# emonosuke/emoASR

Measured on AMD Instinct MI355X. Metric: train frames/sec + decode RTF, Conformer-CTC 23M, 80-mel, 1/2/4/8 GPU, higher is better.
Workload: dtype bf16; 1 GPU; CTC(Conformer) 23M `L2`, bf16, SpecAugment on-GPU, synthetic LibriSpeech-shaped batches (2000 utts, lognormal lengths, ASRBatchSampler packing 30000 frames/50 utts per GPU), one step = accum_grad 5 micro-batches (the reference's accum_grad: 5, asr/train_asr.py:106-128, stacked through the engine in one pass) fwd+bwd, then all-reduce+clip+Adam; dropout 0.1; accum_grad=5, stacked_micro_batches=True, parallelism=dp1

## Files before the change

emoasr_amd/csrc/api.hip:

```cpp
#include <cstdarg>
#include <cstdio>
#include <cstring>
#include <map>
#include <mutex>
#include <tuple>
#include "common.h"
#include "../../include/emoasr_hip.h"

static thread_local char g_err[512] = "";

EmoScratch* emo_stream_scratch(int slot, void* stream, size_t bytes) {
  static std::mutex mu;
  static std::map<std::tuple<int, void*, int>, EmoScratch*> tab;
  int dev = 0;
  if (hipGetDevice(&dev) != hipSuccess) return nullptr;
  std::lock_guard<std::mutex> lock(mu);
  const auto key = std::make_tuple(dev, stream, slot);
  auto it = tab.find(key);
  if (it != tab.end() && it->second->bytes >= bytes) return it->second;
  hipStreamCaptureStatus cap = hipStreamCaptureStatusNone;
  if (hipStreamIsCapturing((hipStream_t)stream, &cap) != hipSuccess || cap != hipStreamCaptureStatusNone) {
    emo_set_error("stream scratch %d: first use on a stream that is being captured (run the call once eagerly on this stream)", slot);
    return nullptr;
  }
  void* d = nullptr;
  if (hipMalloc(&d, bytes) != hipSuccess || hipMemsetAsync(d, 0, bytes, (hipStream_t)stream) != hipSuccess) {
    emo_set_error("stream scratch %d: allocation of %zu bytes failed", slot, bytes);
    return nullptr;
  }
  EmoScratch* r = new EmoScratch{};
  r->dev = d; r->bytes = bytes;
  tab[key] = r;
  return r;
}

void emo_set_error(const char* fmt, ...) {
  va_list ap;
  va_start(ap, fmt);
  vsnprintf(g_err, sizeof(g_err), fmt, ap);
  va_end(ap);
}

void emo_gemm_set_tr_read(int v);
void emo_gemm_set_tile(int v);
void emo_gemm_set_tn_group_blocks(int v);
void emo_gemm_set_tn_group_kb(int v);
void emo_gemm_set_tn_place(int v);
void emo_gemm_set_tn_big(int v);
void emo_gemm_set_tn_big_blocks(int v);
void emo_gemm_set_wholek(int v);
void emo_gemm_set_kb(int v);
void emo_gemm_set_xcd(int v);
void emo_gemm_set_split_tile(int v);
void emo_gemm_set_split_kb(int v);
void emo_gemm_set_split_min128(int v);
void emo_gemm_set_conv_big(int v);
void emo_gemm_set_big_bm(int v);
void emo_gemm_set_big_korder(int v);
void emo_gemm_set_big_min_tiles(int v);
void emo_conv_set_dwconv_lds(int v);
void emo_layer_set_conv_fused(int v);
void emo_layer_set_wgrad_side(int v);
void emo_layer_set_stack_launch(int v);
void emo_layer_set_ffn_save_dact(int v);
void emo_layer_set_att_bits(int v);
void emo_ln_set_fwd8(int v);
void emo_gemm_set_wide128(int v);
void emo_gemm_set_big_n256(int v);
void emo_gemm_set_big_waves(int v);
void emo_conv1_set_pair(int v);
void emo_attn_set_prelaunch(int v);
void emo_ln_set_bwd_pf(int v);
void emo_ln_set_bwd_blocks(int v);
void emo_rnnt_set_greedy_coop(int v);
void emo_rnnt_set_beam_mfma(int v);
void emo_decode_set_coop(int v);
void emo_lstm_set_coop(int v);
void emo_decode_set_coop_merge(int v);
void emo_attn_set_tr_read(int v);
void emo_attn_set_fw(int v);
void emo_attn_set_fwd4(int v);
void emo_attn_set_q2(int v);
void emo_attn_set_bwd_split(int v);
void emo_attn_set_side(int v);
void emo_attn_set_side_prio(int v);
void emo_attn_set_lpt(int v);
void emo_attn_set_fwd_split(int v);
void emo_attn_set_xcd(int v);
void emo_attn_set_fwd_waves(int v);

#include <vector>
namespace {
const char* const kTimerNames[EMO_TIMER_COUNT] = {"attn_bwd_fused_kernel", "attn_bwd_dpos_kernel", "attn_fwd_kernel",
                                                  "gemm_tn_grouped_kernel", "gemm_nt_nn", "gemm_tn", "layernorm", "conv_module"};
struct TimerRec { hipEvent_t e0, e1; double flops, bytes; bool ended; };
std::vector<TimerRec> g_rec[EMO_TIMER_COUNT];
int g_timers_on = 0;
int g_timer_stride = 1;
long g_timer_seen[EMO_TIMER_COUNT];
bool g_timer_open[EMO_TIMER_COUNT];
bool timer_on(int id) { return g_timers_on == 1 || (g_timers_on > 1 && ((g_timers_on >> (id + 1)) & 1)); }
}
void emo_timer_begin(int id, hipStream_t s, double flops, double bytes) {
  if (!timer_on(id)) return;
  g_timer_open[id] = (g_timer_seen[id]++ % g_timer_stride) == 0;
  if (!g_timer_open[id]) return;
  TimerRec r{};
  hipEventCreate(&r.e0);
  hipEventCreate(&r.e1);
  hipEventRecord(r.e0, s);
  r.flops = flops; r.bytes = bytes; r.ended = false;
  g_rec[id].push_back(r);
}
void emo_timer_end(int id, hipStream_t s) {
  if (!timer_on(id) || !g_timer_open[id] || g_rec[id].empty() || g_rec[id].back().ended) return;
  hipEventRecord(g_rec[id].back().e1, s);
  g_rec[id].back().ended = true;
}
extern "C" int emoasr_timer_read_ex(const char* name, int* calls, double* ms, double* flops, double* bytes, int reset) {
  for (int id = 0; id < EMO_TIMER_COUNT; ++id) {
    if (strcmp(name, kTimerNames[id]) != 0) continue;
    double tot = 0.0, fl = 0.0, by = 0.0;
    int n = 0;
    for (const TimerRec& r : g_rec[id]) {
      if (!r.ended) continue;
      float t = 0.f;
      hipEventSynchronize(r.e1);
      if (hipEventElapsedTime(&t, r.e0, r.e1) == hipSuccess) { tot += t; fl += r.flops; by += r.bytes; ++n; }
    }
    if (calls) *calls = n;
    if (ms) *ms = tot;
    if (flops) *flops = fl;
    if (bytes) *bytes = by;
    if (reset) {
      for (const TimerRec& r : g_rec[id]) { hipEventDestroy(r.e0); hipEventDestroy(r.e1); }
      g_rec[id].clear();
    }
    return 0;
  }
  emo_set_error("unknown timer '%s'", name);
  return 1;
}
extern "C" int emoasr_timer_read(const char* name, int* calls, double* ms, int reset) {
  return emoasr_timer_read_ex(name, calls, ms, nullptr, nullptr, reset);
}

extern "C" const char* emoasr_last_error(void) { return g_err; }
extern "C" int emoasr_version(void) { return 1; }
extern "C" int emoasr_set_option(const char* name, int value) {
  if (strcmp(name, "tr_read") == 0) {
    emo_gemm_set_tr_read(value);
    emo_attn_set_tr_read(value);
    return 0;
  }
  if (strcmp(name, "gemm_tile") == 0) { emo_gemm_set_tile(value); return 0; }
  if (strcmp(name, "tn_group_blocks") == 0) { emo_gemm_set_tn_group_blocks(value); return 0; }
  if (strcmp(name, "tn_group_kb") == 0) { emo_gemm_set_tn_group_kb(value); return 0; }
  if (strcmp(name, "tn_place") == 0) { emo_gemm_set_tn_place(value); return 0; }
  if (strcmp(name, "tn_big") == 0) { emo_gemm_set_tn_big(value); return 0; }
  if (strcmp(name, "tn_big_blocks") == 0) { emo_gemm_set_tn_big_blocks(value); return 0; }
  if (strcmp(name, "gemm_wholek") == 0) { emo_gemm_set_wholek(value); return 0; }
  if (strcmp(name, "gemm_kb") == 0) { emo_gemm_set_kb(value); return 0; }
  if (strcmp(name, "gemm_xcd") == 0) { emo_gemm_set_xcd(value); return 0; }
  if (strcmp(name, "split_tile") == 0) { emo_gemm_set_split_tile(value); return 0; }
  if (strcmp(name, "split_kb") == 0) { emo_gemm_set_split_kb(value); return 0; }
  if (strcmp(name, "split_min128") == 0) { emo_gemm_set_split_min128(value); return 0; }
  if (strcmp(name, "conv_big") == 0) { emo_gemm_set_conv_big(value); return 0; }
  if (strcmp(name, "big_bm") == 0) { emo_gemm_set_big_bm(value); return 0; }
  if (strcmp(name, "big_korder") == 0) { emo_gemm_set_big_korder(value); return 0; }
  if (strcmp(name, "big_min_tiles") == 0) { emo_gemm_set_big_min_tiles(value); return 0; }
  if (strcmp(name, "dwconv_lds") == 0) { emo_conv_set_dwconv_lds(value); return 0; }
  if (strcmp(name, "conv_fused") == 0) { emo_layer_set_conv_fused(value); return 0; }
  if (strcmp(name, "wgrad_side") == 0) { emo_layer_set_wgrad_side(value); return 0; }
  if (strcmp(name, "stack_launch") == 0) { emo_layer_set_stack_launch(value); return 0; }
  if (strcmp(name, "ffn_save_dact") == 0) { emo_layer_set_ffn_save_dact(value); return 0; }
  if (strcmp(name, "attn_mask_bits") == 0) { emo_layer_set_att_bits(value); return 0; }
  if (strcmp(name, "attn_prelaunch") == 0) { emo_attn_set_prelaunch(value); return 0; }
  if (strcmp(name, "conv1_pair") == 0) { emo_conv1_set_pair(value); return 0; }
  if (strcmp(name, "big_waves") == 0) { emo_gemm_set_big_waves(value); return 0; }
  if (strcmp(name, "big_n256") == 0) { emo_gemm_set_big_n256(value); return 0; }
  if (strcmp(name, "gemm_wide128") == 0) { emo_gemm_set_wide128(value); return 0; }
  if (strcmp(name, "ln_fwd8") == 0) { emo_ln_set_fwd8(value); return 0; }
  if (strcmp(name, "ln_bwd_pf") == 0) { emo_ln_set_bwd_pf(value); return 0; }
  if (strcmp(name, "ln_bwd_blocks") == 0) { emo_ln_set_bwd_blocks(value); return 0; }
  if (strcmp(name, "rnnt_greedy_coop") == 0) { emo_rnnt_set_greedy_coop(value); return 0; }
  if (strcmp(name, "rnnt_beam_mfma") == 0) { emo_rnnt_set_beam_mfma(value); return 0; }
  if (strcmp(name, "decode_coop") == 0) { emo_decode_set_coop(value); return 0; }
  if (strcmp(name, "lstm_coop") == 0) { emo_lstm_set_coop(value); return 0; }
  if (strcmp(name, "decode_coop_merge") == 0) { emo_decode_set_coop_merge(value); return 0; }
  if (strcmp(name, "attn_fw") == 0) { emo_attn_set_fw(value); return 0; }
  if (strcmp(name, "attn_fwd4") == 0) { emo_attn_set_fwd4(value); return 0; }
  if (strcmp(name, "attn_q2") == 0) { emo_attn_set_q2(value); return 0; }
  if (strcmp(name, "attn_bwd_split") == 0) { emo_attn_set_bwd_split(value); return 0; }
  if (strcmp(name, "attn_side") == 0) { emo_attn_set_side(value); return 0; }
  if (strcmp(name, "attn_side_prio") == 0) { emo_attn_set_side_prio(value); return 0; }
  if (strcmp(name, "attn_lpt") == 0) { emo_attn_set_lpt(value); return 0; }
  if (strcmp(name, "attn_fwd_split") == 0) { emo_attn_set_fwd_split(value); return 0; }
  if (strcmp(name, "attn_xcd") == 0) { emo_attn_set_xcd(value); return 0; }
  if (strcmp(name, "attn_fwd_waves") == 0) { emo_attn_set_fwd_waves(value); return 0; }
  if (strcmp(name, "timers") == 0) { g_timers_on = value; return 0; }
  if (strcmp(name, "timer_stride") == 0) { g_timer_stride = value > 0 ? value : 1; return 0; }
  emo_set_error("unknown option '%s'", name);
  return 1;
}
```

emoasr_amd/csrc/convfused.hip:

```cpp
#include <algorithm>
#include "common.h"
#include "../../include/emoasr_hip.h"

namespace {

constexpr int CF_TT = 32;
constexpr int CF_MAXK = 31;
constexpr int CF_ROWS = CF_TT + CF_MAXK - 1;
constexpr int CF_CB = 256;
constexpr int CF_ROWS_P = 64;

typedef __attribute__((ext_vector_type(2))) float f2;
__device__ __forceinline__ f2 unpack2(unsigned u) { return f2{__uint_as_float(u << 16), __uint_as_float(u & 0xffff0000u)}; }
__device__ __forceinline__ unsigned pack2(f2 v) {
  const bf16 lo = (bf16)v[0], hi = (bf16)v[1];
  return (unsigned)__builtin_bit_cast(unsigned short, lo) | ((unsigned)__builtin_bit_cast(unsigned short, hi) << 16);
}
__device__ __forceinline__ unsigned lds_pair(const bf16* base, int row, int pair) {
  return *reinterpret_cast<const unsigned*>(base + row * CF_CB + 2 * pair);
}

template <bool GLU>
__global__ __launch_bounds__(CF_CB) void cf_dwconv_kernel(int Tn, int C, int K, const bf16* __restrict__ x,
                                                        const float* __restrict__ w, const float* __restrict__ bias,
                                                        bf16* __restrict__ y, int flip, float* __restrict__ part,
                                                        const RowSegs sg) {
  __shared__ __attribute__((aligned(16))) bf16 zs[CF_ROWS_P * CF_CB];
  __shared__ __attribute__((aligned(16))) bf16 os[CF_TT * CF_CB];
  const int tid = threadIdx.x;
  const int cb = blockIdx.y * CF_CB;
  const int ldx = GLU ? 2 * C : C;
  int b = blockIdx.z, nx = gridDim.x;
  if (sg.n > 1) {
    const int si = rowsegs_of_utt(sg, b);
    Tn = sg.T[si];
    x += sg.row[si] * ldx;
    y += sg.row[si] * C;
    if (part) part += sg.part[si];
    b -= sg.b0[si];
    nx = (Tn + CF_TT - 1) / CF_TT;
    if ((int)blockIdx.x >= nx) return;
  }
  const int t0 = blockIdx.x * CF_TT, pad = (K - 1) / 2;
  const int nch = min(CF_CB, C - cb);
  const int pr = tid & (CF_CB / 2 - 1), half = tid / (CF_CB / 2);
  f2 wr[CF_MAXK];
  {
    float* wsm = reinterpret_cast<float*>(zs);
    for (int idx = tid; idx < nch * K; idx += CF_CB) wsm[idx] = w[(long)cb * K + idx];
    __syncthreads();
#pragma unroll
    for (int j = 0; j < CF_MAXK; ++j) {
      const int jj = flip ? K - 1 - j : j;
      wr[j] = (j < K && 2 * pr < nch) ? f2{wsm[(2 * pr) * K + jj], wsm[(2 * pr + 1) * K + jj]} : f2{0.f, 0.f};
    }
    __syncthreads();
  }
  const __amdgpu_buffer_rsrc_t rs = make_rsrc(x + (long)b * Tn * ldx);
  const int ch8 = (tid & (CF_CB / 8 - 1)) * 8;
  {
    Vec16<bf16> sa[CF_ROWS_P / 8], sg[GLU ? CF_ROWS_P / 8 : 1];
#pragma unroll
    for (int it = 0; it < CF_ROWS_P / 8; ++it) {
      const int row = tid / (CF_CB / 8) + it * 8;
      const int t = t0 + row - pad;
      const bool ok = row < CF_TT + K - 1 && t >= 0 && t < Tn && ch8 < nch;
      const unsigned off = ok ? (unsigned)(((long)t * ldx + cb + ch8) * 2) : EMO_OOB;
      sa[it] = buf_load16<bf16>(rs, off);
      if constexpr (GLU) sg[it] = buf_load16<bf16>(rs, ok ? off + (unsigned)(C * 2) : EMO_OOB);
    }
#pragma unroll
    for (int it = 0; it < CF_ROWS_P / 8; ++it) {
      const int row = tid / (CF_CB / 8) + it * 8;
      Vec16<bf16> a = sa[it];
      if constexpr (GLU) {
#pragma unroll
        for (int e = 0; e < 8; ++e) a.v[e] = (bf16)((float)a.v[e] * sigmoidf_((float)sg[it].v[e]));
      }
      store16(&zs[row * CF_CB + ch8], a);
    }
  }
  __syncthreads();
  {
    const int c0 = cb + 2 * pr;
    if (2 * pr < nch) {
      const f2 bv = bias ? f2{bias[c0], bias[c0 + 1]} : f2{0.f, 0.f};
      f2 win[CF_TT / 2 + CF_MAXK - 1];
#pragma unroll
      for (int i = 0; i < CF_TT / 2 + CF_MAXK - 1; ++i) win[i] = unpack2(lds_pair(zs, half * (CF_TT / 2) + i, pr));
#pragma unroll
      for (int i = 0; i < CF_TT / 2; ++i) {
        f2 acc = bv;
#pragma unroll
        for (int j = 0; j < CF_MAXK; ++j) acc = emo_mac2(wr[j], win[i + j], acc);
        *reinterpret_cast<unsigned*>(os + (half * (CF_TT / 2) + i) * CF_CB + 2 * pr) = pack2(acc);
      }
    }
  }
  __syncthreads();
#pragma unroll
  for (int it = 0; it < CF_TT / 8; ++it) {
    const int row = tid / (CF_CB / 8) + it * 8;
    if (t0 + row < Tn && ch8 < nch)
      *reinterpret_cast<bf16x8*>(y + ((long)b * Tn + t0 + row) * C + cb + ch8) = *reinterpret_cast<const bf16x8*>(os + row * CF_CB + ch8);
  }
  if (part && tid < nch) {
    float out[CF_TT];
    float s = 0.f;
#pragma unroll
    for (int i = 0; i < CF_TT; ++i) {
      out[i] = t0 + i < Tn ? (float)os[i * CF_CB + tid] : 0.f;
      s += out[i];
    }
    const int n = min(CF_TT, Tn - t0);
    const float mb = s / n;
    float m2 = 0.f;
#pragma unroll
    for (int i = 0; i < CF_TT; ++i) {
      const float d = out[i] - mb;
      m2 += i < n ? d * d : 0.f;
    }
    float* p = part + ((long)b * nx + blockIdx.x) * 2 * C + cb + tid;
    p[0] = s;
    p[C] = m2;
  }
}

__global__ __launch_bounds__(CF_CB) void cf_conv_bwd_kernel(int Tn, int C, int K, const bf16* __restrict__ ds,
                                                          const bf16* __restrict__ cv, const float* __restrict__ mean,
                                                          const float* __restrict__ var, const float* __restrict__ gamma,
                                                          const float* __restrict__ beta, float eps,
                                                          const float* __restrict__ tot, const bf16* __restrict__ g,
                                                          const float* __restrict__ w, bf16* __restrict__ dg,
                                                          float* __restrict__ wpart, const RowSegs sg) {
  extern __shared__ __attribute__((aligned(16))) char smem[];
  bf16* dcs = reinterpret_cast<bf16*>(smem);
  bf16* zs = dcs + CF_ROWS_P * CF_CB;
  const int tid = threadIdx.x;
  const int cb = blockIdx.y * CF_CB;
  const int nch = min(CF_CB, C - cb);
  int b = blockIdx.z;
  if (sg.n > 1) {
    const int si = rowsegs_of_utt(sg, b);
    Tn = sg.T[si];
    ds += sg.row[si] * C; cv += sg.row[si] * C; g += sg.row[si] * 2 * C; dg += sg.row[si] * 2 * C;
    mean += (long)si * C; var += (long)si * C; tot += (long)si * 2 * C;
    b -= sg.b0[si];
    if ((int)blockIdx.x * CF_TT >= Tn) {
      float* p = wpart + ((long)blockIdx.z * gridDim.x + blockIdx.x) * (K + 1) * C + cb + tid;
      if (tid < nch)
        for (int j = 0; j <= K; ++j) p[(long)j * C] = 0.f;
      return;
    }
  }
  const int t0 = blockIdx.x * CF_TT, pad = (K - 1) / 2;
  const int ch8 = (tid & (CF_CB / 8 - 1)) * 8;
  const bool chok = ch8 < nch;
  const int pr = tid & (CF_CB / 2 - 1), half = tid / (CF_CB / 2);
  f2 wr[CF_MAXK];
  {
    float* wsm = reinterpret_cast<float*>(smem);
    for (int idx = tid; idx < nch * K; idx += CF_CB) wsm[idx] = w[(long)cb * K + idx];
    __syncthreads();
#pragma unroll
    for (int j = 0; j < CF_MAXK; ++j)
      wr[j] = (j < K && 2 * pr < nch) ? f2{wsm[(2 * pr) * K + (K - 1 - j)], wsm[(2 * pr + 1) * K + (K - 1 - j)]} : f2{0.f, 0.f};
    __syncthreads();
  }
  {
    const __amdgpu_buffer_rsrc_t rsd = make_rsrc(ds + (long)b * Tn * C), rsc = make_rsrc(cv + (long)b * Tn * C);
    const __amdgpu_buffer_rsrc_t rsg = make_rsrc(g + (long)b * Tn * 2 * C);
    {
      Vec16<bf16> ga[CF_ROWS_P / 8], gb[CF_ROWS_P / 8];
#pragma unroll
      for (int it = 0; it < CF_ROWS_P / 8; ++it) {
        const int row = tid / (CF_CB / 8) + it * 8;
        const int t = t0 + row - pad;
        const bool ok = row < CF_TT + K - 1 && t >= 0 && t < Tn && chok;
        const unsigned goff = ok ? (unsigned)(((long)t * 2 * C + cb + ch8) * 2) : EMO_OOB;
        ga[it] = buf_load16<bf16>(rsg, goff);
        gb[it] = buf_load16<bf16>(rsg, ok ? goff + (unsigned)(C * 2) : EMO_OOB);
      }
#pragma unroll
      for (int it = 0; it < CF_ROWS_P / 8; ++it) {
        const int row = tid / (CF_CB / 8) + it * 8;
        const int core = row - pad;
        (void)core;
        Vec16<bf16> z;
#pragma unroll
        for (int e = 0; e < 8; ++e) z.v[e] = (bf16)((float)ga[it].v[e] * sigmoidf_((float)gb[it].v[e]));
        store16(&zs[row * CF_CB + ch8], z);
      }
    }
    float mu[8], is[8], gm[8], bt[8], m1[8], m2[8];
#pragma unroll
    for (int j = 0; j < 8; ++j) {
      const int cc = cb + ch8 + j;
      mu[j] = chok ? mean[cc] : 0.f; is[j] = chok ? rsqrtf(var[cc] + eps) : 0.f;
      gm[j] = chok ? gamma[cc] : 0.f; bt[j] = chok ? beta[cc] : 0.f;
      m1[j] = chok ? tot[cc] : 0.f; m2[j] = chok ? tot[C + cc] : 0.f;
    }
    Vec16<bf16> dvs[CF_ROWS_P / 8], yvs[CF_ROWS_P / 8];
#pragma unroll
    for (int it = 0; it < CF_ROWS_P / 8; ++it) {
      const int row = tid / (CF_CB / 8) + it * 8;
      const int t = t0 + row - pad;
      const bool ok = row < CF_TT + K - 1 && t >= 0 && t < Tn && chok;
      const unsigned off = ok ? (unsigned)(((long)t * C + cb + ch8) * 2) : EMO_OOB;
      dvs[it] = buf_load16<bf16>(rsd, off);
      yvs[it] = buf_load16<bf16>(rsc, off);
    }
#pragma unroll
    for (int it = 0; it < CF_ROWS_P / 8; ++it) {
      const int row = tid / (CF_CB / 8) + it * 8;
      const int t = t0 + row - pad;
      const bool ok = row < CF_TT + K - 1 && t >= 0 && t < Tn && chok;
      const Vec16<bf16> dv = dvs[it], yv = yvs[it];
      Vec16<bf16> o;
#pragma unroll
      for (int e = 0; e < 8; ++e) {
        const float xh = ((float)yv.v[e] - mu[e]) * is[e];
        const float dbn = (float)dv.v[e] * dswishf_(gm[e] * xh + bt[e]);
        o.v[e] = ok ? (bf16)(gm[e] * is[e] * (dbn - m1[e] - xh * m2[e])) : (bf16)0.f;
      }
      store16(&dcs[row * CF_CB + ch8], o);
    }
  }
  __syncthreads();
  if (2 * pr >= nch) return;
  const int c0 = cb + 2 * pr;
  {
    f2 dcw[CF_TT / 2 + CF_MAXK - 1];
#pragma unroll
    for (int i = 0; i < CF_TT / 2 + CF_MAXK - 1; ++i) dcw[i] = unpack2(lds_pair(dcs, half * (CF_TT / 2) + i, pr));
    bf16* dgb = dg + (long)b * Tn * 2 * C + c0;
#pragma unroll
    for (int i = 0; i < CF_TT / 2; ++i) {
      f2 acc = f2{0.f, 0.f};
#pragma unroll
      for (int j = 0; j < CF_MAXK; ++j) acc = emo_mac2(wr[j], dcw[i + j], acc);
      const f2 d = unpack2(pack2(acc));
      const int fr = half * (CF_TT / 2) + i;
      const bool fok = t0 + fr < Tn;
      const bf16* gp = g + ((long)b * Tn + (fok ? t0 + fr : 0)) * 2 * C + c0;
      const f2 a = fok ? unpack2(*reinterpret_cast<const unsigned*>(gp)) : f2{0.f, 0.f};
      const f2 gt = fok ? unpack2(*reinterpret_cast<const unsigned*>(gp + C)) : f2{0.f, 0.f};
      const f2 sg = f2{sigmoidf_(gt[0]), sigmoidf_(gt[1])};
      if (t0 + fr < Tn) {
        *reinterpret_cast<unsigned*>(dgb + (long)(t0 + fr) * 2 * C) = pack2(d * sg);
        *reinterpret_cast<unsigned*>(dgb + (long)(t0 + fr) * 2 * C + C) = pack2(d * a * sg * (f2{1.f, 1.f} - sg));
      }
    }
  }
  {
    constexpr int TAPS = (CF_MAXK + 1) / 2;
    const int j0 = half * TAPS;
    f2 dcc[CF_TT];
#pragma unroll
    for (int i = 0; i < CF_TT; ++i) dcc[i] = unpack2(lds_pair(dcs, i + pad, pr));
    f2 zw[CF_TT + TAPS - 1];
#pragma unroll
    for (int i = 0; i < CF_TT + TAPS - 1; ++i) zw[i] = j0 + i < CF_ROWS_P ? unpack2(lds_pair(zs, j0 + i, pr)) : f2{0.f, 0.f};
    f2 acc[TAPS];
#pragma unroll
    for (int j = 0; j < TAPS; ++j) acc[j] = f2{0.f, 0.f};
    f2 sb = f2{0.f, 0.f};
#pragma unroll
    for (int i = 0; i < CF_TT; ++i) {
      const f2 d = dcc[i];
      sb += d;
#pragma unroll
      for (int j = 0; j < TAPS; ++j) acc[j] = emo_mac2(d, zw[i + j], acc[j]);
    }
    const long blk = ((long)blockIdx.z * gridDim.x + blockIdx.x);
    float* p = wpart + blk * (K + 1) * C + c0;
#pragma unroll
    for (int j = 0; j < TAPS; ++j)
      if (j0 + j < K) *reinterpret_cast<f2*>(p + (long)(j0 + j) * C) = acc[j];
    if (half == 0) *reinterpret_cast<f2*>(p + (long)K * C) = sb;
  }
}

}

int emo_dwconv_bwd_w_reduce(int nblk, int C, int K, const float* part, float* dw, float* dbias, hipStream_t s);

extern "C" int emoasr_glu_dwconv_fwd(int dtype, int B, int Tn, int C, int K, const void* g, const float* w,
                                     const float* bias, void* c, float* part, void* stream) {
  EMO_CHECK(dtype == EMO_BF16, "glu_dwconv_fwd: bf16 only");
  EMO_CHECK(K <= CF_MAXK && (K & 1) && C % 8 == 0, "glu_dwconv_fwd: K=%d (odd, <= %d), C=%d (multiple of 8)", K, CF_MAXK, C);
  EMO_CHECK((long)Tn * 2 * C * 2 < (1L << 32), "glu_dwconv_fwd: utterance larger than 4 GiB");
  if (B * Tn == 0) return 0;
  dim3 grid(cdiv(Tn, CF_TT), cdiv(C, CF_CB), B);
  cf_dwconv_kernel<true><<<grid, CF_CB, 0, (hipStream_t)stream>>>(Tn, C, K, (const bf16*)g, w, bias, (bf16*)c, 0, part, RowSegs{});
  EMO_LAUNCH_CHECK();
  return 0;
}

int emo_dwconv_lds(int B, int Tn, int C, int K, const void* x, const float* w, const float* bias, void* y, int flip,
                   float* part, hipStream_t s) {
  dim3 grid(cdiv(Tn, CF_TT), cdiv(C, CF_CB), B);
  cf_dwconv_kernel<false><<<grid, CF_CB, 0, s>>>(Tn, C, K, (const bf16*)x, w, bias, (bf16*)y, flip, part, RowSegs{});
  EMO_LAUNCH_CHECK();
  return 0;
}

extern "C" int emoasr_conv_bwd_fused(int dtype, int B, int Tn, int C, int K, const void* ds, const void* cv,
                                     const float* mean, const float* var, const float* gamma, const float* beta, float eps,
                                     const float* tot, const void* g, const float* w, void* dg, float* dw, float* dbias,
                                     float* scratch, void* stream) {
  EMO_CHECK(dtype == EMO_BF16, "conv_bwd_fused: bf16 only");
  EMO_CHECK(K <= CF_MAXK && (K & 1) && C % 8 == 0, "conv_bwd_fused: K=%d (odd, <= %d), C=%d (multiple of 8)", K, CF_MAXK, C);
  EMO_CHECK((long)Tn * 2 * C * 2 < (1L << 32), "conv_bwd_fused: utterance larger than 4 GiB");
  EMO_CHECK(scratch != nullptr && tot != nullptr, "conv_bwd_fused: scratch and tot are required");
  if (B * Tn == 0) return 0;
  hipStream_t s = (hipStream_t)stream;
  constexpr int bytes = 2 * CF_ROWS_P * CF_CB * 2;
  static bool attr_done = false;
  if (!attr_done) {
    hipError_t e = hipFuncSetAttribute((const void*)cf_conv_bwd_kernel, hipFuncAttributeMaxDynamicSharedMemorySize, bytes);
    if (e != hipSuccess) { emo_set_error("hipFuncSetAttribute(%d): %s", bytes, hipGetErrorString(e)); return 1; }
    attr_done = true;
  }
  dim3 grid(cdiv(Tn, CF_TT), cdiv(C, CF_CB), B);
  cf_conv_bwd_kernel<<<grid, CF_CB, bytes, s>>>(Tn, C, K, (const bf16*)ds, (const bf16*)cv, mean, var, gamma, beta, eps, tot,
                                              (const bf16*)g, w, (bf16*)dg, scratch, RowSegs{});
  EMO_LAUNCH_CHECK();
  return emo_dwconv_bwd_w_reduce(grid.x * B, C, K, scratch, dw, dbias, s);
}

int emo_bn_stats_finalize_seg(const RowSegs& sg, int C, const float* part, float* mean, float* var, float* running_mean,
                              float* running_var, float momentum, long long* nbt, hipStream_t s);
int emo_bn_swish_fwd_seg(const RowSegs& sg, int C, const void* y, const float* mean, const float* var, const float* gamma,
                         const float* beta, float eps, void* z, hipStream_t s);
int emo_bn_swish_bwd_sums_seg(const RowSegs& sg, int C, const void* dz, const void* y, const float* mean, const float* var,
                              const float* gamma, const float* beta, float eps, float* dgamma, float* dbeta, float* scratch,
                              float** tot_out, hipStream_t s);

namespace {
bool row_segs(const emoasr_segments_t* seg, int C, RowSegs* out, int* tmax) {
  if (!seg || seg->n < 1 || seg->n > EMOASR_MAX_SEGMENTS) return false;
  RowSegs sg{};
  sg.n = seg->n;
  *tmax = 0;
  for (int i = 0; i < seg->n; ++i) {
    if (seg->B[i] <= 0 || seg->T[i] <= 0) return false;
    sg.b0[i + 1] = sg.b0[i] + seg->B[i];
    sg.T[i] = seg->T[i];
    sg.row[i + 1] = sg.row[i] + (long)seg->B[i] * seg->T[i];
    sg.part[i + 1] = sg.part[i] + emoasr_dwconv_stats_floats(seg->B[i], seg->T[i], C);
    sg.sums[i + 1] = sg.sums[i] + (emoasr_bn_swish_bwd_scratch_floats(seg->B[i] * seg->T[i], C) / (2 * C) - 1);
    *tmax = std::max(*tmax, seg->T[i]);
  }
  *out = sg;
  return true;
}
}

extern "C" int emoasr_conv_module_fwd_seg(int dtype, const emoasr_segments_t* seg, int C, int K, const void* g, const float* w,
                                          const float* bias, void* c, float* part, float* bmean, float* bvar, float* running_mean,
                                          float* running_var, float momentum, long long* num_batches_tracked, const float* gamma,
                                          const float* beta, float eps, void* z, int training, void* stream) {
  EMO_CHECK(dtype == EMO_BF16, "conv_module_fwd_seg: bf16 only");
  EMO_CHECK(K <= CF_MAXK && (K & 1) && C % 8 == 0, "conv_module_fwd_seg: K=%d (odd, <= %d), C=%d (multiple of 8)", K, CF_MAXK, C);
  RowSegs sg;
  int tmax = 0;
  EMO_CHECK(row_segs(seg, C, &sg, &tmax), "conv_module_fwd_seg: bad segment description");
  EMO_CHECK((long)tmax * 2 * C * 2 < (1L << 32) && sg.row[sg.n] * 2 * C * 2 < (1L << 46), "conv_module_fwd_seg: batch too large");
  EMO_CHECK(!training || (part && bmean && bvar), "conv_module_fwd_seg: training needs the BatchNorm buffers");
  hipStream_t s = (hipStream_t)stream;
  EmoTimerScope timer_(EMO_TIMER_CONV_MODULE, s, 0.0, 5.0 * (double)sg.row[sg.n] * C * 2.0);
  dim3 grid(cdiv(tmax, CF_TT), cdiv(C, CF_CB), sg.b0[sg.n]);
  cf_dwconv_kernel<true><<<grid, CF_CB, 0, s>>>(tmax, C, K, (const bf16*)g, w, bias, (bf16*)c, 0, training ? part : nullptr, sg);
  EMO_LAUNCH_CHECK();
  if (training) {
    if (emo_bn_stats_finalize_seg(sg, C, part, bmean, bvar, running_mean, running_var, momentum, num_batches_tracked, s)) return 1;
    return emo_bn_swish_fwd_seg(sg, C, c, bmean, bvar, gamma, beta, eps, z, s);
  }
  RowSegs one{};
  one.n = 1; one.b0[1] = sg.b0[sg.n]; one.row[1] = sg.row[sg.n];
  return emo_bn_swish_fwd_seg(one, C, c, running_mean, running_var, gamma, beta, eps, z, s);
}

extern "C" long emoasr_conv_module_bwd_seg_scratch_floats(const emoasr_segments_t* seg, int C, int K, int which) {
  RowSegs sg;
  int tmax = 0;
  if (!row_segs(seg, C, &sg, &tmax)) return 0;
  if (which == 0) return (sg.sums[sg.n] + 2 * sg.n) * 2 * C;
  return emoasr_dwconv_bwd_w_scratch_floats(sg.b0[sg.n], tmax, C, K);
}

extern "C" int emoasr_conv_module_bwd_seg(int dtype, const emoasr_segments_t* seg, int C, int K, const void* dz, const void* c,
                                          const float* bmean, const float* bvar, const float* gamma, const float* beta, float eps,
                                          float* dgamma, float* dbeta, const void* g, const float* w, void* dg, float* dw,
                                          float* dbias, float* bn_scratch, float* dw_scratch, void* stream) {
  EMO_CHECK(dtype == EMO_BF16, "conv_module_bwd_seg: bf16 only");
  EMO_CHECK(K <= CF_MAXK && (K & 1) && C % 8 == 0, "conv_module_bwd_seg: K=%d (odd, <= %d), C=%d (multiple of 8)", K, CF_MAXK, C);
  EMO_CHECK(bn_scratch && dw_scratch, "conv_module_bwd_seg: scratch required");
  RowSegs sg;
  int tmax = 0;
  EMO_CHECK(row_segs(seg, C, &sg, &tmax), "conv_module_bwd_seg: bad segment description");
  hipStream_t s = (hipStream_t)stream;
  EmoTimerScope timer_(EMO_TIMER_CONV_MODULE, s, 0.0, 8.0 * (double)sg.row[sg.n] * C * 2.0);
  float* tot = nullptr;
  if (emo_bn_swish_bwd_sums_seg(sg, C, dz, c, bmean, bvar, gamma, beta, eps, dgamma, dbeta, bn_scratch, &tot, s)) return 1;
  constexpr int bytes = 2 * CF_ROWS_P * CF_CB * 2;
  static bool attr_done = false;
  if (!attr_done) {
    hipError_t e = hipFuncSetAttribute((const void*)cf_conv_bwd_kernel, hipFuncAttributeMaxDynamicSharedMemorySize, bytes);
    if (e != hipSuccess) { emo_set_error("hipFuncSetAttribute(%d): %s", bytes, hipGetErrorString(e)); return 1; }
    attr_done = true;
  }
  dim3 grid(cdiv(tmax, CF_TT), cdiv(C, CF_CB), sg.b0[sg.n]);
  cf_conv_bwd_kernel<<<grid, CF_CB, bytes, s>>>(tmax, C, K, (const bf16*)dz, (const bf16*)c, bmean, bvar, gamma, beta, eps, tot,
                                              (const bf16*)g, w, (bf16*)dg, dw_scratch, sg);
  EMO_LAUNCH_CHECK();
  return emo_dwconv_bwd_w_reduce(grid.x * sg.b0[sg.n], C, K, dw_scratch, dw, dbias, s);
}
```

emoasr_amd/csrc/convmodule.hip:

```cpp
#include <algorithm>
#include "common.h"
#include "../../include/emoasr_hip.h"

namespace {

constexpr int DW_TT = 32;
constexpr int DW_MAXK = 31;
constexpr int DW_WCHUNKS = 1;

template <typename T>
__global__ __launch_bounds__(256) void dwconv_kernel(int Tn, int C, int K, const T* __restrict__ x,
                                                     const float* __restrict__ w,
                                                     const float* __restrict__ bias, T* __restrict__ y,
                                                     int flip, float* __restrict__ part, const RowSegs sg) {
  const int c = blockIdx.y * 256 + threadIdx.x;
  if (c >= C) return;
  int b = blockIdx.z;
  if (sg.n > 1) {
    const int si = rowsegs_of_utt(sg, b);
    Tn = sg.T[si];
    x += sg.row[si] * C; y += sg.row[si] * C;
    if (part) part += sg.part[si];
    b -= sg.b0[si];
    if ((int)blockIdx.x * DW_TT >= Tn) return;
  }
  const int nx = (Tn + DW_TT - 1) / DW_TT;
  const int t0 = blockIdx.x * DW_TT, pad = (K - 1) / 2;
  float wr[DW_MAXK];
#pragma unroll
  for (int j = 0; j < DW_MAXK; ++j) wr[j] = j < K ? w[c * K + (flip ? K - 1 - j : j)] : 0.f;
  const float bv = bias ? bias[c] : 0.f;
  float win[DW_TT + DW_MAXK - 1];
  const __amdgpu_buffer_rsrc_t rs = make_rsrc(x + (long)b * Tn * C);
#pragma unroll
  for (int i = 0; i < DW_TT + DW_MAXK - 1; ++i) {
    const int t = t0 + i - pad;
    const bool ok = i < DW_TT + K - 1 && t >= 0 && t < Tn;
    win[i] = buf_load_f32<T>(rs, ok ? (unsigned)(((long)t * C + c) * sizeof(T)) : EMO_OOB);
  }
  T* yb = y + (long)b * Tn * C + c;
  float out[DW_TT];
  float s = 0.f;
#pragma unroll
  for (int i = 0; i < DW_TT; ++i) {
    float acc = bv;
#pragma unroll
    for (int j = 0; j < DW_MAXK; ++j) acc = emo_mac(wr[j], win[i + j], acc);
    const T r = from_f32<T>(acc);
    out[i] = t0 + i < Tn ? to_f32(r) : 0.f;
    s += out[i];
    if (t0 + i < Tn) yb[(long)(t0 + i) * C] = r;
  }
  if (part) {
    const int n = min(DW_TT, Tn - t0);
    const float mb = s / n;
    float m2 = 0.f;
#pragma unroll
    for (int i = 0; i < DW_TT; ++i) {
      const float d = out[i] - mb;
      m2 += i < n ? d * d : 0.f;
    }
    float* p = part + ((long)b * nx + blockIdx.x) * 2 * C + c;
    p[0] = s;
    p[C] = m2;
  }
}

constexpr int BNF_CH = 16, BNF_G = 64;
#define EMO_BN_TICKETS(stream_)                                                                   \
  EmoScratch* tsc_ = emo_stream_scratch(EMO_SCRATCH_BN_TICKETS, (void*)(stream_), 2 * 64 * sizeof(unsigned)); \
  if (!tsc_) return 1;                                                                            \
  unsigned* tickets_ = static_cast<unsigned*>(tsc_->dev)
__global__ __launch_bounds__(1024) void bn_stats_finalize_kernel(int B_, int Tn_, int C, const float* __restrict__ part_,
                                                                 float* __restrict__ mean_, float* __restrict__ var_,
                                                                 float* __restrict__ running_mean,
                                                                 float* __restrict__ running_var, float momentum,
                                                                 long long* __restrict__ num_batches_tracked, const RowSegs sg,
                                                                 unsigned* __restrict__ tickets) {
  __shared__ float red[BNF_G][BNF_CH];
  __shared__ float mean_s[BNF_CH];
  __shared__ int s_last;
  const int lane = threadIdx.x % BNF_CH, grp = threadIdx.x / BNF_CH;
  const int c = blockIdx.x * BNF_CH + lane;
  const int ns = sg.n > 1 ? sg.n : 1, si = blockIdx.y;
  const int B = sg.n > 1 ? sg.b0[si + 1] - sg.b0[si] : B_, Tn = sg.n > 1 ? sg.T[si] : Tn_;
  const float* part = sg.n > 1 ? part_ + sg.part[si] : part_;
  float* mean = mean_ + (long)si * C;
  float* var = var_ + (long)si * C;
  const int nx = (Tn + DW_TT - 1) / DW_TT, nblk = B * nx;
  const float M = (float)B * Tn;
  float s = 0.f;
  if (c < C) {
#pragma unroll 8
    for (int k = grp; k < nblk; k += BNF_G) s += part[(long)k * 2 * C + c];
  }
  red[grp][lane] = s;
  __syncthreads();
  if (grp == 0) {
    float t = 0.f;
#pragma unroll
    for (int g = 0; g < BNF_G; ++g) t += red[g][lane];
    mean_s[lane] = t / M;
  }
  __syncthreads();
  const float mu = mean_s[lane];
  float m2 = 0.f;
  if (c < C)
#pragma unroll 8
    for (int k = grp; k < nblk; k += BNF_G) {
      const int n = min(DW_TT, Tn - (k % nx) * DW_TT);
      const float d = part[(long)k * 2 * C + c] / n - mu;
      m2 += part[(long)k * 2 * C + C + c] + n * d * d;
    }
  __syncthreads();
  red[grp][lane] = m2;
  __syncthreads();
  float m2sum = 0.f;
  if (grp == 0 && c < C) {
#pragma unroll
    for (int g = 0; g < BNF_G; ++g) m2sum += red[g][lane];
    mean[c] = mu;
    var[c] = m2sum / M;
  }
  if (!running_mean && !running_var && !num_batches_tracked) return;
  __syncthreads();
  if (threadIdx.x == 0) {
    __threadfence();
    s_last = atomicAdd(&tickets[blockIdx.x], 1u) == (unsigned)ns - 1;
  }
  __syncthreads();
  if (!s_last) return;
  __threadfence();
  if (grp == 0 && c < C) {
    float rm = running_mean ? running_mean[c] : 0.f, rv = running_var ? running_var[c] : 0.f;
    for (int k = 0; k < ns; ++k) {
      const float Mk = sg.n > 1 ? (float)(sg.row[k + 1] - sg.row[k]) : M;
      const float mk = __hip_atomic_load(mean_ + (long)k * C + c, __ATOMIC_RELAXED, __HIP_MEMORY_SCOPE_AGENT);
      const float vk = __hip_atomic_load(var_ + (long)k * C + c, __ATOMIC_RELAXED, __HIP_MEMORY_SCOPE_AGENT);
      const float m2k = k == si ? m2sum : vk * Mk;
      rm = (1.f - momentum) * rm + momentum * (k == si ? mu : mk);
      rv = (1.f - momentum) * rv + momentum * (Mk > 1.f ? m2k / (Mk - 1.f) : m2k / Mk);
    }
    if (running_mean) running_mean[c] = rm;
    if (running_var) running_var[c] = rv;
  }
  if (threadIdx.x == 0) {
    tickets[blockIdx.x] = 0u;
    if (num_batches_tracked && blockIdx.x == 0) *num_batches_tracked += ns;
  }
}

template <typename T>
__global__ __launch_bounds__(256) void dwconv_bwd_w_kernel(int Tn, int C, int K, const T* __restrict__ dy,
                                                           const T* __restrict__ x, float* __restrict__ part, const RowSegs sg) {
  const int c = blockIdx.y * 256 + threadIdx.x;
  if (c >= C) return;
  int b = blockIdx.z;
  const int pad = (K - 1) / 2;
  if (sg.n > 1) {
    const int si = rowsegs_of_utt(sg, b);
    Tn = sg.T[si];
    x += sg.row[si] * C; dy += sg.row[si] * C;
    b -= sg.b0[si];
  }
  float acc[DW_MAXK];
#pragma unroll
  for (int j = 0; j < DW_MAXK; ++j) acc[j] = 0.f;
  float sb = 0.f;
  const __amdgpu_buffer_rsrc_t rsx = make_rsrc(x + (long)b * Tn * C), rsd = make_rsrc(dy + (long)b * Tn * C);
  for (int cc = 0; cc < DW_WCHUNKS; ++cc) {
    const int t0 = (blockIdx.x * DW_WCHUNKS + cc) * DW_TT;
    if (t0 >= Tn) break;
    float win[DW_TT + DW_MAXK - 1];
#pragma unroll
    for (int i = 0; i < DW_TT + DW_MAXK - 1; ++i) {
      const int t = t0 + i - pad;
      const bool ok = i < DW_TT + K - 1 && t >= 0 && t < Tn;
      win[i] = buf_load_f32<T>(rsx, ok ? (unsigned)(((long)t * C + c) * sizeof(T)) : EMO_OOB);
    }
    float dv[DW_TT];
#pragma unroll
    for (int i = 0; i < DW_TT; ++i)
      dv[i] = buf_load_f32<T>(rsd, t0 + i < Tn ? (unsigned)(((long)(t0 + i) * C + c) * sizeof(T)) : EMO_OOB);
#pragma unroll
    for (int i = 0; i < DW_TT; ++i) {
      const float d = dv[i];
      sb += d;
#pragma unroll
      for (int j = 0; j < DW_MAXK; ++j) acc[j] = emo_mac(d, win[i + j], acc[j]);
    }
  }
  const long blk = ((long)blockIdx.z * gridDim.x + blockIdx.x);
  float* p = part + blk * (K + 1) * C + c;
#pragma unroll
  for (int j = 0; j < DW_MAXK; ++j)
    if (j < K) p[(long)j * C] = acc[j];
  p[(long)K * C] = sb;
}

__global__ __launch_bounds__(256) void dwconv_bwd_w_reduce_kernel(int nblk, int C, int K,
                                                                  const float* __restrict__ part,
                                                                  float* __restrict__ dw,
                                                                  float* __restrict__ dbias) {
  __shared__ float red[4][64];
  const int lane = threadIdx.x & 63, wave = threadIdx.x >> 6;
  const int i = blockIdx.x * 64 + lane;
  const int n = (K + 1) * C;
  const int per = (nblk + gridDim.y - 1) / gridDim.y;
  const int b0 = blockIdx.y * per, b1 = min(nblk, b0 + per);
  float s = 0.f;
  if (i < n) {
#pragma unroll 8
    for (int b = b0 + wave; b < b1; b += 4) s += part[(long)b * n + i];
  }
  red[wave][lane] = s;
  __syncthreads();
  if (wave == 0 && i < n) {
    s = red[0][lane] + red[1][lane] + red[2][lane] + red[3][lane];
    const int j = i / C, c = i % C;
    if (gridDim.y == 1) {
      if (j < K) dw[c * K + j] += s;
      else if (dbias) dbias[c] += s;
    } else {
      if (j < K) atomicAdd(&dw[c * K + j], s);
      else if (dbias) atomicAdd(&dbias[c], s);
    }
  }
}

constexpr int BN_ROWS = 16;
constexpr int BN_STAT_ROWS = 64;
template <typename T>
__global__ __launch_bounds__(256) void bn_sum_kernel(int M, int C, const T* __restrict__ y,
                                                     float* __restrict__ sum) {
  const int c = blockIdx.x * 256 + threadIdx.x;
  if (c >= C) return;
  const int r0 = blockIdx.y * BN_STAT_ROWS, r1 = min(M, r0 + BN_STAT_ROWS);
  float s = 0.f;
  for (int r = r0; r < r1; ++r) s += to_f32(y[(long)r * C + c]);
  atomicAdd(&sum[c], s);
}
template <typename T>
__global__ __launch_bounds__(256) void bn_var_kernel(int M, int C, const T* __restrict__ y,
                                                     const float* __restrict__ sum,
                                                     float* __restrict__ sq) {
  const int c = blockIdx.x * 256 + threadIdx.x;
  if (c >= C) return;
  const float mu = sum[c] / M;
  const int r0 = blockIdx.y * BN_STAT_ROWS, r1 = min(M, r0 + BN_STAT_ROWS);
  float s = 0.f;
  for (int r = r0; r < r1; ++r) { const float d = to_f32(y[(long)r * C + c]) - mu; s += d * d; }
  atomicAdd(&sq[c], s);
}
__global__ void bn_finalize_kernel(int M, int C, float* mean, float* var, float* running_mean,
                                   float* running_var, float momentum) {
  const int c = blockIdx.x * 256 + threadIdx.x;
  if (c >= C) return;
  const float mu = mean[c] / M, vb = var[c] / M;
  mean[c] = mu; var[c] = vb;
  if (running_mean) running_mean[c] = (1.f - momentum) * running_mean[c] + momentum * mu;
  if (running_var) {
    const float vu = M > 1 ? var[c] * M / (M - 1) : vb;
    running_var[c] = (1.f - momentum) * running_var[c] + momentum * vu;
  }
}

template <typename T>
__global__ __launch_bounds__(256) void bn_swish_fwd_kernel(long n, int C, const T* __restrict__ y,
                                                           const float* __restrict__ mean,
                                                           const float* __restrict__ var,
                                                           const float* __restrict__ gamma,
                                                           const float* __restrict__ beta, float eps,
                                                           T* __restrict__ z, const RowSegs sg) {
  for (long i = (long)blockIdx.x * 256 + threadIdx.x; i < n; i += (long)gridDim.x * 256) {
    const int c = i % C;
    const long so = sg.n > 1 ? (long)rowsegs_of_row(sg, i / C) * C : 0;
    const float xh = (to_f32(y[i]) - mean[so + c]) * rsqrtf(var[so + c] + eps);
    z[i] = from_f32<T>(swish_t<T>(gamma[c] * xh + beta[c]));
  }
}
template <typename T>
__global__ __launch_bounds__(256) void bn_swish_fwd8_kernel(long n8, int C, const T* __restrict__ y,
                                                            const float* __restrict__ mean,
                                                            const float* __restrict__ var,
                                                            const float* __restrict__ gamma,
                                                            const float* __restrict__ beta, float eps,
                                                            T* __restrict__ z, const RowSegs sg) {
  const int cg = C / 8;
  for (long i = (long)blockIdx.x * 256 + threadIdx.x; i < n8; i += (long)gridDim.x * 256) {
    const long row = i / cg;
    const int c = (int)(i - row * cg) * 8;
    const long so = sg.n > 1 ? (long)rowsegs_of_row(sg, row) * C : 0;
    float v[8];
    load8<T>(y + i * 8, v);
#pragma unroll
    for (int j = 0; j < 8; ++j) {
      const float xh = (v[j] - mean[so + c + j]) * rsqrtf(var[so + c + j] + eps);
      v[j] = swish_t<T>(gamma[c + j] * xh + beta[c + j]);
    }
    store8<T>(z + i * 8, v);
  }
}

constexpr int BN_SUM_ROWS = 64;
constexpr int BN_APPLY_ROWS = 16;

template <typename T>
__global__ __launch_bounds__(256) void bn_bwd_sums_kernel(int M, int C, const T* __restrict__ dz,
                                                          const T* __restrict__ y,
                                                          const float* __restrict__ mean,
                                                          const float* __restrict__ var,
                                                          const float* __restrict__ gamma,
                                                          const float* __restrict__ beta, float eps,
                                                          float* __restrict__ part, const RowSegs sg) {
  __shared__ float red[8][2][256];
  const int hl = threadIdx.x & 31, rl = threadIdx.x >> 5;
  const int c = blockIdx.x * 256 + hl * 8;
  const bool cok = c < C;
  long rbase = 0;
  if (sg.n > 1) {
    const int si = blockIdx.z;
    rbase = sg.row[si];
    M = (int)(sg.row[si + 1] - rbase);
    if ((int)blockIdx.y * BN_SUM_ROWS >= M) return;
    mean += (long)si * C; var += (long)si * C;
    part += sg.sums[si] * 2 * C;
  }
  float mu[8], is[8], g[8], bt[8], s1[8], s2[8];
#pragma unroll
  for (int j = 0; j < 8; ++j) {
    mu[j] = cok ? mean[c + j] : 0.f; is[j] = cok ? rsqrtf(var[c + j] + eps) : 0.f;
    g[j] = cok ? gamma[c + j] : 0.f; bt[j] = cok ? beta[c + j] : 0.f;
    s1[j] = 0.f; s2[j] = 0.f;
  }
  const __amdgpu_buffer_rsrc_t rsy = make_rsrc(y), rsd = make_rsrc(dz);
  const int r0 = blockIdx.y * BN_SUM_ROWS;
#pragma unroll 4
  for (int it = 0; it < BN_SUM_ROWS / 8; ++it) {
    const int r = r0 + rl + 8 * it;
    const bool ok = cok && r < M;
    float yv[8], dv[8];
    buf_load8<T>(rsy, (rbase + r) * C + c, ok, yv);
    buf_load8<T>(rsd, (rbase + r) * C + c, ok, dv);
#pragma unroll
    for (int j = 0; j < 8; ++j) {
      const float xh = (yv[j] - mu[j]) * is[j];
      const float dbn = dv[j] * dswish_t<T>(g[j] * xh + bt[j]);
      s1[j] += dbn; s2[j] += dbn * xh;
    }
  }
#pragma unroll
  for (int j = 0; j < 8; ++j) { red[rl][0][hl * 8 + j] = s1[j]; red[rl][1][hl * 8 + j] = s2[j]; }
  __syncthreads();
  const int cc = blockIdx.x * 256 + threadIdx.x;
  if (cc < C) {
    float a = 0.f, b = 0.f;
#pragma unroll
    for (int k = 0; k < 8; ++k) { a += red[k][0][threadIdx.x]; b += red[k][1][threadIdx.x]; }
    part[(long)blockIdx.y * 2 * C + cc] = a;
    part[(long)blockIdx.y * 2 * C + C + cc] = b;
  }
}
__global__ __launch_bounds__(1024) void bn_bwd_fold_kernel(int npart_, int C, float inv_m_, const float* __restrict__ part_,
                                                           float* __restrict__ tot_, float* __restrict__ dgamma,
                                                           float* __restrict__ dbeta, const RowSegs sg,
                                                           unsigned* __restrict__ tickets) {
  __shared__ float red[2][64][16];
  __shared__ int s_last;
  const int lane = threadIdx.x % 16, grp = threadIdx.x / 16;
  const int c = blockIdx.x * 16 + lane;
  const int ns = sg.n > 1 ? sg.n : 1, si = blockIdx.y;
  const int npart = sg.n > 1 ? (int)(sg.sums[si + 1] - sg.sums[si]) : npart_;
  const float inv_m = sg.n > 1 ? 1.f / (float)(sg.row[si + 1] - sg.row[si]) : inv_m_;
  const float* part = sg.n > 1 ? part_ + sg.sums[si] * 2 * C : part_;
  float* tot = tot_ + (long)si * 2 * C;
  float* raw = tot_ + (long)ns * 2 * C + (long)si * 2 * C;
  float a = 0.f, b = 0.f;
  if (c < C) {
#pragma unroll 8
    for (int k = grp; k < npart; k += 64) { a += part[(long)k * 2 * C + c]; b += part[(long)k * 2 * C + C + c]; }
  }
  red[0][grp][lane] = a;
  red[1][grp][lane] = b;
  __syncthreads();
  if (grp == 0 && c < C) {
    a = 0.f; b = 0.f;
#pragma unroll
    for (int g = 0; g < 64; ++g) { a += red[0][g][lane]; b += red[1][g][lane]; }
    tot[c] = a * inv_m;
    tot[C + c] = b * inv_m;
    if (ns == 1) {
      if (dbeta) dbeta[c] += a;
      if (dgamma) dgamma[c] += b;
    } else {
      raw[c] = a;
      raw[C + c] = b;
    }
  }
  if (ns == 1 || (!dbeta && !dgamma)) return;
  __syncthreads();
  if (threadIdx.x == 0) {
    __threadfence();
    s_last = atomicAdd(&tickets[64 + blockIdx.x], 1u) == (unsigned)ns - 1;
  }
  __syncthreads();
  if (!s_last) return;
  __threadfence();
  if (grp == 0 && c < C) {
    float da = 0.f, db = 0.f;
    const float* r0 = tot_ + (long)ns * 2 * C;
    for (int k = 0; k < ns; ++k) {
      da += __hip_atomic_load(r0 + (long)k * 2 * C + c, __ATOMIC_RELAXED, __HIP_MEMORY_SCOPE_AGENT);
      db += __hip_atomic_load(r0 + (long)k * 2 * C + C + c, __ATOMIC_RELAXED, __HIP_MEMORY_SCOPE_AGENT);
    }
    if (dbeta) dbeta[c] += da;
    if (dgamma) dgamma[c] += db;
  }
  if (threadIdx.x == 0) tickets[64 + blockIdx.x] = 0u;
}
template <typename T>
__global__ __launch_bounds__(256) void bn_bwd_apply_kernel(int M, int C, const T* __restrict__ dz,
                                                           const T* __restrict__ y,
                                                           const float* __restrict__ mean,
                                                           const float* __restrict__ var,
                                                           const float* __restrict__ gamma,
                                                           const float* __restrict__ beta, float eps,
                                                           const float* __restrict__ tot,
                                                           T* __restrict__ dy, const RowSegs sg) {
  const int hl = threadIdx.x & 31, rl = threadIdx.x >> 5;
  const int c = blockIdx.x * 256 + hl * 8;
  if (c >= C) return;
  if (sg.n > 1) {
    const int si = blockIdx.z;
    M = (int)(sg.row[si + 1] - sg.row[si]);
    if ((int)blockIdx.y * BN_APPLY_ROWS >= M) return;
    dz += sg.row[si] * C; y += sg.row[si] * C; dy += sg.row[si] * C;
    mean += (long)si * C; var += (long)si * C; tot += (long)si * 2 * C;
  }
  float mu[8], is[8], g[8], bt[8], m1[8], m2[8];
#pragma unroll
  for (int j = 0; j < 8; ++j) {
    mu[j] = mean[c + j]; is[j] = rsqrtf(var[c + j] + eps); g[j] = gamma[c + j]; bt[j] = beta[c + j];
    m1[j] = tot[c + j]; m2[j] = tot[C + c + j];
  }
  const __amdgpu_buffer_rsrc_t rsy = make_rsrc(y), rsd = make_rsrc(dz);
  const int r0 = blockIdx.y * BN_APPLY_ROWS;
#pragma unroll
  for (int it = 0; it < BN_APPLY_ROWS / 8; ++it) {
    const int r = r0 + rl + 8 * it;
    const bool ok = r < M;
    float yv[8], dv[8], o[8];
    buf_load8<T>(rsy, (long)r * C + c, ok, yv);
    buf_load8<T>(rsd, (long)r * C + c, ok, dv);
#pragma unroll
    for (int j = 0; j < 8; ++j) {
      const float xh = (yv[j] - mu[j]) * is[j];
      const float dbn = dv[j] * dswish_t<T>(g[j] * xh + bt[j]);
      o[j] = g[j] * is[j] * (dbn - m1[j] - xh * m2[j]);
    }
    if (ok) store8<T>(dy + (long)r * C + c, o);
  }
}

inline int ew_grid(long n) { long b = (n + 255) / 256; return (int)(b > 8192 ? 8192 : (b < 1 ? 1 : b)); }

}

int emo_dwconv_lds(int B, int Tn, int C, int K, const void* x, const float* w, const float* bias, void* y, int flip,
                   float* part, hipStream_t s);
static int g_dwconv_lds = 1;
void emo_conv_set_dwconv_lds(int v) { g_dwconv_lds = v; }
static bool use_lds(int dtype, int Tn, int C) {
  return g_dwconv_lds && dtype == EMO_BF16 && C % 8 == 0 && (long)Tn * C * 2 < (1L << 32);
}
int emo_dwconv_bwd_w_reduce(int nblk, int C, int K, const float* part, float* dw, float* dbias, hipStream_t s) {
  dwconv_bwd_w_reduce_kernel<<<dim3(cdiv((K + 1) * C, 64), nblk >= 1024 ? 4 : 1), 256, 0, s>>>(nblk, C, K, part, dw, dbias);
  EMO_LAUNCH_CHECK();
  return 0;
}

extern "C" int emoasr_dwconv_fwd(int dtype, int B, int Tn, int C, int K, const void* x, const float* w,
                                 const float* bias, void* y, void* stream) {
  EMO_CHECK(K <= DW_MAXK && (K & 1), "dwconv: K=%d unsupported (odd, <= %d)", K, DW_MAXK);
  if (B * Tn == 0) return 0;
  if (use_lds(dtype, Tn, C)) return emo_dwconv_lds(B, Tn, C, K, x, w, bias, y, 0, nullptr, (hipStream_t)stream);
  dim3 grid(cdiv(Tn, DW_TT), cdiv(C, 256), B);
  EMO_DISPATCH(dtype, (dwconv_kernel<T><<<grid, 256, 0, (hipStream_t)stream>>>(Tn, C, K, (const T*)x, w,
                                                                              bias, (T*)y, 0, nullptr, RowSegs{})));
  EMO_LAUNCH_CHECK();
  return 0;
}

extern "C" long emoasr_dwconv_stats_floats(int B, int Tn, int C) { return (long)B * cdiv(Tn, DW_TT) * 2 * C; }

extern "C" int emoasr_dwconv_fwd_stats(int dtype, int B, int Tn, int C, int K, const void* x, const float* w,
                                       const float* bias, void* y, float* part, void* stream) {
  EMO_CHECK(K <= DW_MAXK && (K & 1), "dwconv: K=%d unsupported", K);
  EMO_CHECK(part != nullptr && B * Tn > 0, "dwconv_fwd_stats: needs a non-empty batch and the partials buffer");
  if (use_lds(dtype, Tn, C)) return emo_dwconv_lds(B, Tn, C, K, x, w, bias, y, 0, part, (hipStream_t)stream);
  dim3 grid(cdiv(Tn, DW_TT), cdiv(C, 256), B);
  EMO_DISPATCH(dtype, (dwconv_kernel<T><<<grid, 256, 0, (hipStream_t)stream>>>(Tn, C, K, (const T*)x, w,
                                                                              bias, (T*)y, 0, part, RowSegs{})));
  EMO_LAUNCH_CHECK();
  return 0;
}

extern "C" int emoasr_bn_stats_finalize(int B, int Tn, int C, const float* part, float* mean, float* var,
                                        float* running_mean, float* running_var, float momentum,
                                        long long* num_batches_tracked, void* stream) {
  EMO_CHECK(B * Tn > 0, "bn_stats_finalize: empty batch");
  EMO_CHECK(cdiv(C, BNF_CH) <= 64, "bn_stats_finalize: C=%d too wide for the ticket table", C);
  EMO_BN_TICKETS(stream);
  bn_stats_finalize_kernel<<<cdiv(C, BNF_CH), 1024, 0, (hipStream_t)stream>>>(B, Tn, C, part, mean, var, running_mean,
                                                                          running_var, momentum, num_batches_tracked, RowSegs{}, tickets_);
  EMO_LAUNCH_CHECK();
  return 0;
}
extern "C" int emoasr_dwconv_bwd_x(int dtype, int B, int Tn, int C, int K, const void* dy, const float* w,
                                   void* dx, void* stream) {
  EMO_CHECK(K <= DW_MAXK && (K & 1), "dwconv: K=%d unsupported", K);
  if (B * Tn == 0) return 0;
  if (use_lds(dtype, Tn, C)) return emo_dwconv_lds(B, Tn, C, K, dy, w, nullptr, dx, 1, nullptr, (hipStream_t)stream);
  dim3 grid(cdiv(Tn, DW_TT), cdiv(C, 256), B);
  EMO_DISPATCH(dtype, (dwconv_kernel<T><<<grid, 256, 0, (hipStream_t)stream>>>(Tn, C, K, (const T*)dy, w,
                                                                              nullptr, (T*)dx, 1, nullptr, RowSegs{})));
  EMO_LAUNCH_CHECK();
  return 0;
}
extern "C" long emoasr_dwconv_bwd_w_scratch_floats(int B, int Tn, int C, int K) {
  return (long)B * cdiv(Tn, DW_TT * DW_WCHUNKS) * (K + 1) * C;
}

extern "C" int emoasr_dwconv_bwd_w(int dtype, int B, int Tn, int C, int K, const void* dy, const void* x,
                                   float* dw, float* dbias, int accumulate, float* scratch, void* stream) {
  EMO_CHECK(K <= DW_MAXK && (K & 1), "dwconv: K=%d unsupported", K);
  hipStream_t s = (hipStream_t)stream;
  if (!accumulate) {
    hipMemsetAsync(dw, 0, sizeof(float) * C * K, s);
    if (dbias) hipMemsetAsync(dbias, 0, sizeof(float) * C, s);
  }
  if (B * Tn == 0) return 0;
  EMO_CHECK(scratch != nullptr, "dwconv_bwd_w: scratch of emoasr_dwconv_bwd_w_scratch_floats() floats required");
  dim3 grid(cdiv(Tn, DW_TT * DW_WCHUNKS), cdiv(C, 256), B);
  EMO_DISPATCH(dtype, (dwconv_bwd_w_kernel<T><<<grid, 256, 0, s>>>(Tn, C, K, (const T*)dy, (const T*)x, scratch, RowSegs{})));
  const int nblk = grid.x * B;
  dwconv_bwd_w_reduce_kernel<<<cdiv((K + 1) * C, 64), 256, 0, s>>>(nblk, C, K, scratch, dw, dbias);
  EMO_LAUNCH_CHECK();
  return 0;
}

extern "C" int emoasr_bn_stats(int dtype, int M, int C, const void* y, float* mean, float* var,
                               float* running_mean, float* running_var, float momentum, void* stream) {
  EMO_CHECK(M > 0, "bn_stats: empty batch");
  hipStream_t s = (hipStream_t)stream;
  hipMemsetAsync(mean, 0, sizeof(float) * C, s);
  hipMemsetAsync(var, 0, sizeof(float) * C, s);
  dim3 grid(cdiv(C, 256), cdiv(M, BN_STAT_ROWS));
  EMO_DISPATCH(dtype, (bn_sum_kernel<T><<<grid, 256, 0, s>>>(M, C, (const T*)y, mean)));
  EMO_DISPATCH(dtype, (bn_var_kernel<T><<<grid, 256, 0, s>>>(M, C, (const T*)y, mean, var)));
  bn_finalize_kernel<<<cdiv(C, 256), 256, 0, s>>>(M, C, mean, var, running_mean, running_var, momentum);
  EMO_LAUNCH_CHECK();
  return 0;
}

extern "C" int emoasr_bn_swish_fwd(int dtype, int M, int C, const void* y, const float* mean,
                                   const float* var, const float* gamma, const float* beta, float eps,
                                   void* z, void* stream) {
  const long n = (long)M * C;
  if (n == 0) return 0;
  if (C % 8 == 0 && (reinterpret_cast<uintptr_t>(y) | reinterpret_cast<uintptr_t>(z)) % 16 == 0) {
    EMO_DISPATCH(dtype, (bn_swish_fwd8_kernel<T><<<ew_grid(n / 8), 256, 0, (hipStream_t)stream>>>(
                            n / 8, C, (const T*)y, mean, var, gamma, beta, eps, (T*)z, RowSegs{})));
  } else {
    EMO_DISPATCH(dtype, (bn_swish_fwd_kernel<T><<<ew_grid(n), 256, 0, (hipStream_t)stream>>>(
                            n, C, (const T*)y, mean, var, gamma, beta, eps, (T*)z, RowSegs{})));
  }
  EMO_LAUNCH_CHECK();
  return 0;
}

extern "C" long emoasr_bn_swish_bwd_scratch_floats(int M, int C) { return ((long)cdiv(M, BN_SUM_ROWS) + 1) * 2 * C; }

extern "C" int emoasr_bn_swish_bwd_sums(int dtype, int M, int C, const void* dz, const void* y, const float* mean,
                                        const float* var, const float* gamma, const float* beta, float eps,
                                        float* dgamma, float* dbeta, float* scratch, float** tot_out, void* stream) {
  EMO_CHECK(M > 0, "bn_swish_bwd_sums: empty batch");
  hipStream_t s = (hipStream_t)stream;
  EMO_CHECK(C % 8 == 0, "bn_swish_bwd_sums: C=%d must be a multiple of 8", C);
  EMO_CHECK((long)M * C * (dtype == EMO_BF16 ? 2 : 4) < (1L << 32), "bn_swish_bwd_sums: activation larger than 4 GiB");
  const int npart = cdiv(M, BN_SUM_ROWS);
  dim3 sgrid(cdiv(C, 256), npart);
  EMO_DISPATCH(dtype, (bn_bwd_sums_kernel<T><<<sgrid, 256, 0, s>>>(M, C, (const T*)dz, (const T*)y, mean,
                                                                  var, gamma, beta, eps, scratch, RowSegs{})));
  float* tot = scratch + (long)npart * 2 * C;
  EMO_BN_TICKETS(s);
  bn_bwd_fold_kernel<<<cdiv(C, 16), 1024, 0, s>>>(npart, C, 1.f / M, scratch, tot, dgamma, dbeta, RowSegs{}, tickets_);
  if (tot_out) *tot_out = tot;
  EMO_LAUNCH_CHECK();
  return 0;
}

extern "C" int emoasr_bn_swish_bwd(int dtype, int M, int C, const void* dz, const void* y,
                                   const float* mean, const float* var, const float* gamma,
                                   const float* beta, float eps, void* dy, float* dgamma, float* dbeta,
                                   float* scratch, void* stream) {
  EMO_CHECK(M > 0, "bn_swish_bwd: empty batch");
  hipStream_t s = (hipStream_t)stream;
  EMO_CHECK(C % 8 == 0, "bn_swish_bwd: C=%d must be a multiple of 8", C);
  EMO_CHECK((long)M * C * (dtype == EMO_BF16 ? 2 : 4) < (1L << 32), "bn_swish_bwd: activation larger than 4 GiB");
  const int npart = cdiv(M, BN_SUM_ROWS);
  dim3 grid(cdiv(C, 256), cdiv(M, BN_APPLY_ROWS));
  dim3 sgrid(cdiv(C, 256), npart);
  EMO_DISPATCH(dtype, (bn_bwd_sums_kernel<T><<<sgrid, 256, 0, s>>>(M, C, (const T*)dz, (const T*)y, mean,
                                                                  var, gamma, beta, eps, scratch, RowSegs{})));
  float* tot = scratch + (long)npart * 2 * C;
  EMO_BN_TICKETS(s);
  bn_bwd_fold_kernel<<<cdiv(C, 16), 1024, 0, s>>>(npart, C, 1.f / M, scratch, tot, dgamma, dbeta, RowSegs{}, tickets_);
  EMO_DISPATCH(dtype, (bn_bwd_apply_kernel<T><<<grid, 256, 0, s>>>(M, C, (const T*)dz, (const T*)y, mean,
                                                                  var, gamma, beta, eps, tot, (T*)dy, RowSegs{})));
  EMO_LAUNCH_CHECK();
  return 0;
}

int emo_bn_stats_finalize_seg(const RowSegs& sg, int C, const float* part, float* mean, float* var, float* running_mean,
                              float* running_var, float momentum, long long* nbt, hipStream_t s) {
  EMO_CHECK(cdiv(C, BNF_CH) <= 64, "bn_stats_finalize: C=%d too wide for the ticket table", C);
  EMO_BN_TICKETS(s);
  bn_stats_finalize_kernel<<<dim3(cdiv(C, BNF_CH), sg.n > 1 ? sg.n : 1), 1024, 0, s>>>(sg.b0[1], sg.T[0], C, part, mean, var,
                                                                                     running_mean, running_var, momentum, nbt, sg, tickets_);
  EMO_LAUNCH_CHECK();
  return 0;
}

int emo_bn_swish_fwd_seg_dt(int dtype, const RowSegs& sg, int C, const void* y, const float* mean, const float* var,
                            const float* gamma, const float* beta, float eps, void* z, hipStream_t s) {
  const long n = sg.row[sg.n] * C;
  if (n == 0) return 0;
  if (C % 8 == 0) {
    EMO_DISPATCH(dtype, (bn_swish_fwd8_kernel<T><<<ew_grid(n / 8), 256, 0, s>>>(n / 8, C, (const T*)y, mean, var, gamma, beta, eps, (T*)z, sg)));
  } else {
    EMO_DISPATCH(dtype, (bn_swish_fwd_kernel<T><<<ew_grid(n), 256, 0, s>>>(n, C, (const T*)y, mean, var, gamma, beta, eps, (T*)z, sg)));
  }
  EMO_LAUNCH_CHECK();
  return 0;
}
int emo_bn_swish_fwd_seg(const RowSegs& sg, int C, const void* y, const float* mean, const float* var, const float* gamma,
                         const float* beta, float eps, void* z, hipStream_t s) {
  return emo_bn_swish_fwd_seg_dt(EMO_BF16, sg, C, y, mean, var, gamma, beta, eps, z, s);
}
int emo_bn_bwd_apply(int dtype, int M, int C, const void* dz, const void* y, const float* mean, const float* var, const float* gamma,
                     const float* beta, float eps, const float* tot, void* dy, hipStream_t s) {
  dim3 grid(cdiv(C, 256), cdiv(M, BN_APPLY_ROWS));
  EMO_DISPATCH(dtype, (bn_bwd_apply_kernel<T><<<grid, 256, 0, s>>>(M, C, (const T*)dz, (const T*)y, mean, var, gamma, beta, eps, tot, (T*)dy, RowSegs{})));
  EMO_LAUNCH_CHECK();
  return 0;
}
int emo_bn_bwd_apply_seg(int dtype, const RowSegs& sg, int C, const void* dz, const void* y, const float* mean, const float* var,
                         const float* gamma, const float* beta, float eps, const float* tot, void* dy, hipStream_t s) {
  long mmax = 0;
  for (int i = 0; i < sg.n; ++i) mmax = std::max(mmax, sg.row[i + 1] - sg.row[i]);
  dim3 grid(cdiv(C, 256), cdiv((int)mmax, BN_APPLY_ROWS), sg.n);
  EMO_DISPATCH(dtype, (bn_bwd_apply_kernel<T><<<grid, 256, 0, s>>>((int)mmax, C, (const T*)dz, (const T*)y, mean, var, gamma, beta, eps,
                                                                  tot, (T*)dy, sg)));
  EMO_LAUNCH_CHECK();
  return 0;
}
int emo_dwconv_seg(int dtype, const RowSegs& sg, int tmax, int C, int K, const void* x, const float* w, const float* bias, void* y,
                   int flip, float* part, hipStream_t s) {
  EMO_CHECK(K <= DW_MAXK && (K & 1), "dwconv: K=%d unsupported (odd, <= %d)", K, DW_MAXK);
  if (sg.b0[sg.n] == 0 || tmax == 0) return 0;
  dim3 grid(cdiv(tmax, DW_TT), cdiv(C, 256), sg.b0[sg.n]);
  EMO_DISPATCH(dtype, (dwconv_kernel<T><<<grid, 256, 0, s>>>(tmax, C, K, (const T*)x, w, bias, (T*)y, flip, part, sg)));
  EMO_LAUNCH_CHECK();
  return 0;
}
int emo_dwconv_bwd_w_seg(int dtype, const RowSegs& sg, int tmax, int C, int K, const void* dy, const void* x, float* dw, float* dbias,
                         float* scratch, hipStream_t s) {
  EMO_CHECK(K <= DW_MAXK && (K & 1), "dwconv: K=%d unsupported", K);
  if (sg.b0[sg.n] == 0 || tmax == 0) return 0;
  EMO_CHECK(scratch != nullptr, "dwconv_bwd_w_seg: scratch of emoasr_dwconv_bwd_w_scratch_floats(all utterances, longest) floats required");
  dim3 grid(cdiv(tmax, DW_TT * DW_WCHUNKS), cdiv(C, 256), sg.b0[sg.n]);
  EMO_DISPATCH(dtype, (dwconv_bwd_w_kernel<T><<<grid, 256, 0, s>>>(tmax, C, K, (const T*)dy, (const T*)x, scratch, sg)));
  const int nblk = grid.x * sg.b0[sg.n];
  dwconv_bwd_w_reduce_kernel<<<dim3(cdiv((K + 1) * C, 64), nblk >= 1024 ? 4 : 1), 256, 0, s>>>(nblk, C, K, scratch, dw, dbias);
  EMO_LAUNCH_CHECK();
  return 0;
}

int emo_bn_swish_bwd_sums_seg_dt(int dtype, const RowSegs& sg, int C, const void* dz, const void* y, const float* mean, const float* var,
                                 const float* gamma, const float* beta, float eps, float* dgamma, float* dbeta, float* scratch,
                                 float** tot_out, hipStream_t s);
int emo_bn_swish_bwd_sums_seg(const RowSegs& sg, int C, const void* dz, const void* y, const float* mean, const float* var,
                              const float* gamma, const float* beta, float eps, float* dgamma, float* dbeta, float* scratch,
                              float** tot_out, hipStream_t s) {
  return emo_bn_swish_bwd_sums_seg_dt(EMO_BF16, sg, C, dz, y, mean, var, gamma, beta, eps, dgamma, dbeta, scratch, tot_out, s);
}
int emo_bn_swish_bwd_sums_seg_dt(int dtype, const RowSegs& sg, int C, const void* dz, const void* y, const float* mean, const float* var,
                                 const float* gamma, const float* beta, float eps, float* dgamma, float* dbeta, float* scratch,
                                 float** tot_out, hipStream_t s) {
  long mmax = 0;
  for (int i = 0; i < sg.n; ++i) mmax = std::max(mmax, sg.row[i + 1] - sg.row[i]);
  EMO_CHECK(sg.row[sg.n] * C * (dtype == EMO_BF16 ? 2 : 4) < (1L << 32), "bn_swish_bwd_sums_seg: activation larger than 4 GiB");
  dim3 sgrid(cdiv(C, 256), cdiv((int)mmax, BN_SUM_ROWS), sg.n);
  EMO_DISPATCH(dtype, (bn_bwd_sums_kernel<T><<<sgrid, 256, 0, s>>>((int)mmax, C, (const T*)dz, (const T*)y, mean, var, gamma, beta, eps,
                                                                  scratch, sg)));
  float* tot = scratch + sg.sums[sg.n] * 2 * C;
  EMO_CHECK(cdiv(C, 16) <= 64, "bn_swish_bwd_sums_seg: C=%d too wide for the ticket table", C);
  EMO_BN_TICKETS(s);
  bn_bwd_fold_kernel<<<dim3(cdiv(C, 16), sg.n > 1 ? sg.n : 1), 1024, 0, s>>>((int)sg.sums[1], C, 1.f / (float)sg.row[1], scratch, tot,
                                                                         dgamma, dbeta, sg, tickets_);
  if (tot_out) *tot_out = tot;
  EMO_LAUNCH_CHECK();
  return 0;
}
```

emoasr_amd/csrc/layer.hip:

```cpp
#include <math.h>
#include <algorithm>
#include <map>
#include <mutex>
#include <utility>
#include "common.h"
#include "../../include/emoasr_hip.h"

void emo_attn_bwd_fused_extras(float* zero, long zn, const float* cast_src, void* cast_dst, long cn);
void emo_attn_bwd_defer_join(int v);
void emo_attn_bwd_join(void* stream);
int emo_attn_bwd_prelaunch(int dtype, const emoasr_attn_t* a, void* ws, size_t ws_bytes, float* zero, long zn, void* stream);

int emo_bn_stats_finalize_seg(const RowSegs& sg, int C, const float* part, float* mean, float* var, float* running_mean,
                              float* running_var, float momentum, long long* nbt, hipStream_t s);
int emo_bn_swish_fwd_seg_dt(int dtype, const RowSegs& sg, int C, const void* y, const float* mean, const float* var,
                            const float* gamma, const float* beta, float eps, void* z, hipStream_t s);
int emo_bn_swish_bwd_sums_seg_dt(int dtype, const RowSegs& sg, int C, const void* dz, const void* y, const float* mean, const float* var,
                                 const float* gamma, const float* beta, float eps, float* dgamma, float* dbeta, float* scratch,
                                 float** tot_out, hipStream_t s);
int emo_bn_bwd_apply_seg(int dtype, const RowSegs& sg, int C, const void* dz, const void* y, const float* mean, const float* var,
                         const float* gamma, const float* beta, float eps, const float* tot, void* dy, hipStream_t s);
int emo_dwconv_seg(int dtype, const RowSegs& sg, int tmax, int C, int K, const void* x, const float* w, const float* bias, void* y,
                   int flip, float* part, hipStream_t s);
int emo_dwconv_bwd_w_seg(int dtype, const RowSegs& sg, int tmax, int C, int K, const void* dy, const void* x, float* dw, float* dbias,
                         float* scratch, hipStream_t s);

namespace {

emoasr_epilogue_t plain_ep() {
  emoasr_epilogue_t e{};
  e.alpha = 1.f;
  e.res_scale = 1.f;
  return e;
}

int g_att_bits = 1;
int g_ffn_save_dact = 1;
int g_stack_launch = 1;
int g_conv_fused = 1;
bool conv_fused_ok(int dtype, int d) { return g_conv_fused && dtype == EMO_BF16 && d % 8 == 0; }

int g_wgrad_side = 0;
struct WgSide {
  hipStream_t side = nullptr;
  hipEvent_t fork = nullptr, done[2] = {nullptr, nullptr};
  bool pending[2] = {false, false};
  unsigned n = 0;
};
std::mutex g_wg_mu;
std::map<std::pair<int, hipStream_t>, WgSide> g_wg;

WgSide* wg_side_of(hipStream_t s, bool create) {
  hipStreamCaptureStatus cap = hipStreamCaptureStatusNone;
  if (hipStreamIsCapturing(s, &cap) != hipSuccess || cap != hipStreamCaptureStatusNone) return nullptr;
  int dev = 0;
  if (hipGetDevice(&dev) != hipSuccess) return nullptr;
  std::lock_guard<std::mutex> lk(g_wg_mu);
  auto it = g_wg.find({dev, s});
  if (it != g_wg.end()) return &it->second;
  if (!create) return nullptr;
  WgSide w;
  if (hipStreamCreateWithFlags(&w.side, hipStreamNonBlocking) != hipSuccess) return nullptr;
  if (hipEventCreateWithFlags(&w.fork, hipEventDisableTiming) != hipSuccess ||
      hipEventCreateWithFlags(&w.done[0], hipEventDisableTiming) != hipSuccess ||
      hipEventCreateWithFlags(&w.done[1], hipEventDisableTiming) != hipSuccess)
    return nullptr;
  return &(g_wg[{dev, s}] = w);
}

int ffn_fwd(int dtype, int M, int d, int F, const emoasr_ffn_params_t& p, const void* x, float res_scale,
            float p_enc, uint64_t s_in, uint64_t s_out, const emoasr_ffn_stash_t& st, void* stream) {
  if (emoasr_layernorm_fwd(dtype, M, d, x, p.ln_g, p.ln_b, 1e-5f, st.h, st.mean, st.rstd, stream)) return 1;
  emoasr_epilogue_t e1 = plain_ep();
  e1.bias = p.b1; e1.act = EMOASR_ACT_SWISH | (g_ffn_save_dact ? EMOASR_ACT_SAVE_DACT : 0); e1.pre_out = st.u; e1.drop_p = p_enc; e1.seed = s_in;
  if (emoasr_gemm_nt(dtype, M, F, d, st.h, d, p.w1, d, st.a, F, &e1, stream)) return 1;
  emoasr_epilogue_t e2 = plain_ep();
  e2.bias = p.b2; e2.residual = x; e2.ldr = d; e2.res_scale = res_scale; e2.drop_p = p_enc; e2.seed = s_out;
  return emoasr_gemm_nt(dtype, M, d, F, st.a, F, p.w2, F, st.y, d, &e2, stream);
}

struct SegView {
  int n = 0, Btot = 0;
  int B[EMOASR_MAX_SEGMENTS], T[EMOASR_MAX_SEGMENTS], b0[EMOASR_MAX_SEGMENTS];
  long row[EMOASR_MAX_SEGMENTS + 1], prow[EMOASR_MAX_SEGMENTS + 1], part[EMOASR_MAX_SEGMENTS + 1];
  long M() const { return row[n]; }
  long R() const { return prow[n]; }
};

bool seg_view(const emoasr_conformer_fwd_t* io, int d, SegView* v) {
  const emoasr_segments_t& s = io->seg;
  if (s.n < 0 || s.n > EMOASR_MAX_SEGMENTS) return false;
  v->n = s.n > 0 ? s.n : 1;
  v->row[0] = v->prow[0] = v->part[0] = 0;
  v->Btot = 0;
  for (int i = 0; i < v->n; ++i) {
    v->B[i] = s.n > 0 ? s.B[i] : io->B;
    v->T[i] = s.n > 0 ? s.T[i] : io->T;
    if (v->B[i] <= 0 || v->T[i] <= 0) return false;
    v->b0[i] = v->Btot;
    v->Btot += v->B[i];
    v->row[i + 1] = v->row[i] + (long)v->B[i] * v->T[i];
    v->prow[i + 1] = v->prow[i] + 2L * v->T[i] - 1;
    v->part[i + 1] = v->part[i] + emoasr_dwconv_stats_floats(v->B[i], v->T[i], d);
  }
  return true;
}

RowSegs row_segs_of(const SegView& sv, int C) {
  RowSegs sg{};
  sg.n = sv.n;
  for (int i = 0; i < sv.n; ++i) {
    sg.b0[i + 1] = sg.b0[i] + sv.B[i];
    sg.T[i] = sv.T[i];
    sg.row[i + 1] = sv.row[i + 1];
    sg.part[i + 1] = sv.part[i + 1];
    sg.sums[i + 1] = sg.sums[i] + (emoasr_bn_swish_bwd_scratch_floats(sv.B[i] * sv.T[i], C) / (2 * C) - 1);
  }
  return sg;
}

void attn_args_for(emoasr_attn_t& a, const SegView& sv, int s0, int s1, int H, int d, size_t esz, const void* qkv, const void* pp,
                   const int* klens, uint64_t seed) {
  const size_t ro = (size_t)sv.row[s0];
  const char* base = (const char*)qkv + ro * 3 * d * esz;
  int nb = 0, tmax = 0;
  for (int k = s0; k < s1; ++k) { nb += sv.B[k]; tmax = std::max(tmax, sv.T[k]); }
  a.B = nb; a.H = H; a.DK = d / H; a.Tq = tmax; a.Tk = tmax;
  a.ldq = a.ldk = a.ldv = 3 * d; a.ldo = d; a.ldp = d;
  a.q = base; a.k = base + (size_t)d * esz; a.v = base + (size_t)2 * d * esz;
  a.pos = (const char*)pp + (size_t)sv.prow[s0] * d * esz;
  a.klens = klens ? klens + sv.b0[s0] : nullptr;
  a.causal = 0; a.scale = 1.f / sqrtf((float)(d / H));
  a.seed = seed + 0x9E3779B97F4A7C15ull * (uint64_t)s0;
  a.nseg = 0;
  if (s1 - s0 > 1) {
    a.nseg = s1 - s0;
    for (int k = s0; k <= s1; ++k) {
      a.seg_b0[k - s0] = k < s1 ? sv.b0[k] - sv.b0[s0] : nb;
      a.seg_row[k - s0] = sv.row[k] - sv.row[s0];
      a.seg_prow[k - s0] = sv.prow[k] - sv.prow[s0];
      if (k < s1) a.seg_T[k - s0] = sv.T[k];
    }
  }
}

}

void emo_layer_set_wgrad_side(int v) { g_wgrad_side = v ? 1 : 0; }
extern "C" int emoasr_wgrad_side_join(int keep, void* stream) {
  hipStream_t s = (hipStream_t)stream;
  WgSide* w = wg_side_of(s, false);
  if (!w) return 0;
  for (int back = 2; back > (keep > 0 ? 1 : 0); --back) {
    if (w->n < (unsigned)back) continue;
    const int slot = (w->n - back) & 1;
    if (!w->pending[slot]) continue;
    if (hipStreamWaitEvent(s, w->done[slot], 0) != hipSuccess) { emo_set_error("wgrad_side_join: hipStreamWaitEvent failed"); return 1; }
    w->pending[slot] = false;
  }
  return 0;
}
void emo_layer_set_conv_fused(int v) { g_conv_fused = v; }
void emo_layer_set_stack_launch(int v) { g_stack_launch = v; }
void emo_layer_set_ffn_save_dact(int v) { g_ffn_save_dact = v ? 1 : 0; }
void emo_layer_set_att_bits(int v) { g_att_bits = v ? 1 : 0; }

extern "C" int emoasr_conformer_attn_masks(int dtype, int nl, const emoasr_segments_t* seg, int B, int T, int H, int d, const int* klens,
                                           float p_att, const uint64_t* seeds, unsigned* masks, long layer_stride_words, int nw,
                                           void* stream) {
  EMO_CHECK(seg && seeds && masks && nl >= 0 && H > 0 && d % H == 0, "conformer_attn_masks: bad arguments");
  if (p_att <= 0.f) return 0;
  emoasr_conformer_fwd_t io{};
  io.B = B; io.T = T; io.seg = *seg;
  SegView sv;
  EMO_CHECK(seg_view(&io, d, &sv), "conformer_attn_masks: bad batch / segment shapes");
  const size_t esz = dtype == EMO_BF16 ? 2 : 4;
  const int astep = g_stack_launch ? sv.n : 1;
  for (int l = 0; l < nl; ++l)
    for (int si = 0; si < sv.n; si += astep) {
      emoasr_attn_t am{};
      attn_args_for(am, sv, si, si + astep, H, d, esz, nullptr, nullptr, klens, seeds[l]);
      am.drop_p = p_att;
      if (emoasr_attn_dropmask(dtype, &am, masks + (size_t)l * layer_stride_words + (size_t)sv.row[si] * H * nw, nw, stream)) return 1;
    }
  return 0;
}

extern "C" int emoasr_conformer_layer_fwd(int dtype, const emoasr_conformer_layer_t* L,
                                          const emoasr_conformer_fwd_t* io, void* stream) {
  EMO_CHECK(L && io && io->x && io->pos_t, "conformer_layer_fwd: missing arguments");
  const int d = L->d, H = L->H, F = L->F;
  EMO_CHECK(d > 0 && H > 0 && d % H == 0, "conformer_layer_fwd: bad dims d=%d H=%d", d, H);
  SegView sv;
  EMO_CHECK(seg_view(io, d, &sv), "conformer_layer_fwd: bad batch / segment shapes (B=%d T=%d segments=%d)", io->B, io->T, io->seg.n);
  const int M = (int)sv.M(), R = (int)sv.R();
  const size_t esz = dtype == EMO_BF16 ? 2 : 4;
  const float p_enc = io->p_enc;
  const bool att_bits = g_att_bits && io->att_mask && io->training && io->p_att > 0.f && dtype == EMO_BF16;
  const int astep_m = g_stack_launch ? sv.n : 1;
  for (int si = 0; si < sv.n && att_bits && !io->att_mask_ready; si += astep_m) {
    emoasr_attn_t am{};
    attn_args_for(am, sv, si, si + astep_m, H, d, esz, io->qkv, io->pp, io->klens, io->seed[2]);
    am.drop_p = io->p_att;
    if (emoasr_attn_dropmask(dtype, &am, io->att_mask + (size_t)sv.row[si] * H * io->att_mask_nw, io->att_mask_nw, stream)) return 1;
  }
  if (ffn_fwd(dtype, M, d, F, L->ffm, io->x, 0.5f, p_enc, io->seed[0], io->seed[1], io->ffm, stream)) return 1;
  const void* x1 = io->ffm.y;
  if (emoasr_layernorm_fwd(dtype, M, d, x1, L->att_ln_g, L->att_ln_b, 1e-5f, io->at_h, io->at_mean, io->at_rstd, stream))
    return 1;
  {
    emoasr_epilogue_t e = plain_ep();
    e.bias = L->bqkv;
    if (emoasr_gemm_nt(dtype, M, 3 * d, d, io->at_h, d, L->wqkv, d, io->qkv, 3 * d, &e, stream)) return 1;
    emoasr_epilogue_t ep = plain_ep();
    if (emoasr_gemm_nt(dtype, R, d, d, io->pos_t, d, L->wpos, d, io->pp, d, &ep, stream)) return 1;
    const int astep = g_stack_launch ? sv.n : 1;
    for (int si = 0; si < sv.n; si += astep) {
      const size_t ro = (size_t)sv.row[si];
      emoasr_attn_t a{};
      attn_args_for(a, sv, si, si + astep, H, d, esz, io->qkv, io->pp, io->klens, io->seed[2]);
      a.bias_u = L->bias_u; a.bias_v = L->bias_v; a.drop_p = io->p_att;
      a.out = (char*)io->o + ro * d * esz; a.lse = io->lse + ro * H;
      if (att_bits) { a.keep_mask = io->att_mask + ro * H * io->att_mask_nw; a.keep_nw = io->att_mask_nw; }
      if (emoasr_attn_fwd(dtype, &a, stream)) return 1;
    }
    emoasr_epilogue_t eo = plain_ep();
    eo.bias = L->bout; eo.residual = x1; eo.ldr = d; eo.drop_p = p_enc; eo.seed = io->seed[3];
    if (emoasr_gemm_nt(dtype, M, d, d, io->o, d, L->wout, d, io->at_y, d, &eo, stream)) return 1;
  }
  const void* x2 = io->at_y;
  if (emoasr_layernorm_fwd(dtype, M, d, x2, L->cv_ln_g, L->cv_ln_b, 1e-5f, io->cv_h, io->cv_mean, io->cv_rstd, stream))
    return 1;
  {
    emoasr_epilogue_t e = plain_ep();
    e.bias = L->pw1_b;
    if (emoasr_gemm_nt(dtype, M, 2 * d, d, io->cv_h, d, L->pw1, d, io->g, 2 * d, &e, stream)) return 1;
    const bool fused = conv_fused_ok(dtype, d);
    if (!fused && emoasr_glu_fwd(dtype, M, d, io->g, io->gl, stream)) return 1;
    if (io->training) EMO_CHECK(io->bn_part && io->bmean && io->bvar, "conformer_layer_fwd: training needs the BatchNorm buffers");
    const bool conv_one_launch = fused && sv.n > 1 && g_stack_launch;
    if (conv_one_launch &&
        emoasr_conv_module_fwd_seg(dtype, &io->seg, d, L->K, io->g, L->dw_w, L->dw_b, io->c, io->bn_part, io->bmean, io->bvar,
                                   L->bn_rm, L->bn_rv, 0.1f, L->bn_nbt, L->bn_g, L->bn_b, 1e-5f, io->z, io->training, stream))
      return 1;
    const bool bn_one_launch = !fused && io->training && sv.n > 1 && g_stack_launch;
    if (bn_one_launch) {
      const RowSegs sg = row_segs_of(sv, d);
      int tmax = 0;
      for (int si = 0; si < sv.n; ++si) tmax = std::max(tmax, sv.T[si]);
      if (emo_dwconv_seg(dtype, sg, tmax, d, L->K, io->gl, L->dw_w, L->dw_b, io->c, 0, io->bn_part, (hipStream_t)stream)) return 1;
      if (emo_bn_stats_finalize_seg(sg, d, io->bn_part, io->bmean, io->bvar, L->bn_rm, L->bn_rv, 0.1f, L->bn_nbt, (hipStream_t)stream))
        return 1;
      if (emo_bn_swish_fwd_seg_dt(dtype, sg, d, io->c, io->bmean, io->bvar, L->bn_g, L->bn_b, 1e-5f, io->z, (hipStream_t)stream)) return 1;
    }
    for (int si = 0; si < sv.n && !conv_one_launch && !bn_one_launch; ++si) {
      const size_t ro = (size_t)sv.row[si];
      const int B = sv.B[si], T = sv.T[si];
      const char* g = (const char*)io->g + ro * 2 * d * esz;
      const char* gl = io->gl ? (const char*)io->gl + ro * d * esz : nullptr;
      char* c = (char*)io->c + ro * d * esz;
      const float *bmean = L->bn_rm, *bvar = L->bn_rv;
      if (io->training) {
        float* part = io->bn_part + sv.part[si];
        if (fused) {
          if (emoasr_glu_dwconv_fwd(dtype, B, T, d, L->K, g, L->dw_w, L->dw_b, c, part, stream)) return 1;
        } else if (emoasr_dwconv_fwd_stats(dtype, B, T, d, L->K, gl, L->dw_w, L->dw_b, c, part, stream)) {
          return 1;
        }
        if (emoasr_bn_stats_finalize(B, T, d, part, io->bmean + (size_t)si * d, io->bvar + (size_t)si * d, L->bn_rm, L->bn_rv, 0.1f,
                                     L->bn_nbt, stream))
          return 1;
        bmean = io->bmean + (size_t)si * d; bvar = io->bvar + (size_t)si * d;
      } else if (fused) {
        if (emoasr_glu_dwconv_fwd(dtype, B, T, d, L->K, g, L->dw_w, L->dw_b, c, nullptr, stream)) return 1;
      } else if (emoasr_dwconv_fwd(dtype, B, T, d, L->K, gl, L->dw_w, L->dw_b, c, stream)) {
        return 1;
      }
      if (emoasr_bn_swish_fwd(dtype, B * T, d, c, bmean, bvar, L->bn_g, L->bn_b, 1e-5f, (char*)io->z + ro * d * esz, stream)) return 1;
    }
    emoasr_epilogue_t eo = plain_ep();
    eo.bias = L->pw2_b; eo.residual = x2; eo.ldr = d; eo.drop_p = p_enc; eo.seed = io->seed[4];
    if (emoasr_gemm_nt(dtype, M, d, d, io->z, d, L->pw2, d, io->cv_y, d, &eo, stream)) return 1;
  }
  if (ffn_fwd(dtype, M, d, F, L->ff, io->cv_y, 0.5f, p_enc, io->seed[5], io->seed[6], io->ff, stream)) return 1;
  return emoasr_layernorm_fwd(dtype, M, d, io->ff.y, L->fin_ln_g, L->fin_ln_b, 1e-5f, io->y, io->fin_mean, io->fin_rstd, stream);
}

namespace {

struct BwdLayout {
  size_t off = 0;
  size_t take(size_t bytes) { const size_t o = off; off += (bytes + 255) / 256 * 256; return o; }
};

struct BwdBufs {
  size_t dx1, dx2, dx3, dx4, pre1, pre2, pre3, pre4, dh, du_ff, du_ffm, dz, dc, dgl, dg, dout, dqkv, dpos_t;
  size_t dpos, delta, bn_scr, dw_scr, attn_ws, attn_ws_bytes, total;
  size_t img[EMOASR_MAX_SEGMENTS + 1];
};

BwdBufs bwd_layout(int dtype, const SegView& sv, int d, int H, int F, int K) {
  const size_t esz = dtype == EMO_BF16 ? 2 : 4, M = (size_t)sv.M(), R = (size_t)sv.R();
  BwdLayout L;
  BwdBufs b{};
  b.dx1 = L.take(M * d * esz); b.dx2 = L.take(M * d * esz); b.dx3 = L.take(M * d * esz); b.dx4 = L.take(M * d * esz);
  b.pre1 = L.take(M * d * esz); b.pre2 = L.take(M * d * esz); b.pre3 = L.take(M * d * esz); b.pre4 = L.take(M * d * esz);
  b.dh = L.take(M * d * esz);
  b.du_ff = L.take(M * F * esz); b.du_ffm = L.take(M * F * esz);
  b.dz = L.take(M * d * esz); b.dc = L.take(M * d * esz); b.dgl = L.take(M * d * esz); b.dg = L.take(M * 2 * d * esz);
  b.dout = L.take(M * d * esz); b.dqkv = L.take(M * 3 * d * esz); b.dpos_t = L.take(R * d * esz);
  b.dpos = L.take(R * d * 4); b.delta = L.take(M * H * 4);
  size_t bn_scr = 0, dw_scr = 0, attn_ws = 0;
  int tmax = 0;
  for (int i = 0; i < sv.n; ++i) {
    bn_scr = std::max(bn_scr, (size_t)emoasr_bn_swish_bwd_scratch_floats(sv.B[i] * sv.T[i], d) * 4);
    dw_scr = std::max(dw_scr, (size_t)emoasr_dwconv_bwd_w_scratch_floats(sv.B[i], sv.T[i], d, K) * 4);
    attn_ws = std::max(attn_ws, dtype == EMO_BF16 ? emoasr_attn_bwd_fused_ws_bytes(dtype, sv.B[i], H, sv.T[i], sv.T[i], 1)
                                                  : emoasr_attn_bwd_mat_bytes(dtype, sv.B[i], H, sv.T[i], sv.T[i], 1, 1));
    tmax = std::max(tmax, sv.T[i]);
    b.img[i + 1] = b.img[i] + (dtype == EMO_BF16 ? 0 : emoasr_attn_bwd_mat_bytes(dtype, sv.B[i], H, sv.T[i], sv.T[i], 1, 0));
  }
  if (dtype == EMO_BF16)
    attn_ws = std::max(attn_ws, emoasr_attn_bwd_fused_ws_bytes_rows(dtype, (long)M, H, tmax, 1));
  if (sv.n > 1) {
    emoasr_segments_t sg{};
    sg.n = sv.n;
    for (int i = 0; i < sv.n; ++i) { sg.B[i] = sv.B[i]; sg.T[i] = sv.T[i]; }
    bn_scr = std::max(bn_scr, (size_t)emoasr_conv_module_bwd_seg_scratch_floats(&sg, d, K, 0) * 4);
    dw_scr = std::max(dw_scr, (size_t)emoasr_conv_module_bwd_seg_scratch_floats(&sg, d, K, 1) * 4);
  }
  b.bn_scr = L.take(bn_scr);
  b.dw_scr = L.take(dw_scr);
  b.attn_ws_bytes = attn_ws;
  b.attn_ws = L.take(b.attn_ws_bytes);
  b.total = L.off;
  return b;
}

}

extern "C" size_t emoasr_conformer_layer_bwd_ws_bytes_seg(int dtype, const emoasr_segments_t* seg, int d, int H, int F, int K) {
  emoasr_conformer_fwd_t io{};
  if (!seg) return 0;
  io.seg = *seg;
  SegView sv;
  if (seg->n < 1 || !seg_view(&io, d, &sv)) return 0;
  return bwd_layout(dtype, sv, d, H, F, K).total;
}

extern "C" size_t emoasr_conformer_layer_bwd_img_bytes_seg(int dtype, const emoasr_segments_t* seg, int d, int H) {
  emoasr_conformer_fwd_t io{};
  if (!seg || dtype == EMO_BF16) return 0;
  io.seg = *seg;
  SegView sv;
  if (seg->n < 1 || !seg_view(&io, d, &sv)) return 0;
  return bwd_layout(dtype, sv, d, H, 4 * d, 1).img[sv.n];
}

extern "C" size_t emoasr_conformer_layer_bwd_ws_bytes(int dtype, int B, int T, int d, int H, int F, int K) {
  emoasr_segments_t seg{};
  seg.n = 1; seg.B[0] = B; seg.T[0] = T;
  return emoasr_conformer_layer_bwd_ws_bytes_seg(dtype, &seg, d, H, F, K);
}

extern "C" int emoasr_conformer_layer_bwd(int dtype, const emoasr_conformer_layer_t* L, const emoasr_conformer_layer_t* G,
                                          const emoasr_conformer_fwd_t* st, const emoasr_conformer_bwd_t* io, void* stream) {
  EMO_CHECK(L && G && st && io && io->dy && io->dx && io->ws && io->ln_part, "conformer_layer_bwd: missing arguments");
  const int d = L->d, H = L->H, F = L->F, K = L->K;
  SegView sv;
  EMO_CHECK(seg_view(st, d, &sv), "conformer_layer_bwd: bad batch / segment shapes");
  const int M = (int)sv.M(), R = (int)sv.R();
  const BwdBufs bb = bwd_layout(dtype, sv, d, H, F, K);
  EMO_CHECK(io->ws_bytes >= bb.total, "conformer_layer_bwd: workspace %zu < %zu bytes", io->ws_bytes, bb.total);
  char* ws = static_cast<char*>(io->ws);
  const size_t esz = dtype == EMO_BF16 ? 2 : 4;
  EMO_CHECK(dtype == EMO_BF16 || (io->attn_img && io->attn_img_bytes >= bb.img[sv.n]),
            "conformer_layer_bwd: f32 needs the zero-filled attention image area (%zu bytes, emoasr_conformer_layer_bwd_img_bytes_seg)",
            bb.img[sv.n]);
  const float p = st->p_enc;
  hipStream_t s = (hipStream_t)stream;
  emoasr_tn_problem_t pr[EMOASR_TN_GROUP_MAX];
  int npr = 0;
  WgSide* wgs = g_wgrad_side ? wg_side_of(s, true) : nullptr;
  if (wgs && wgs->pending[wgs->n & 1]) {
    if (hipStreamWaitEvent(s, wgs->done[wgs->n & 1], 0) != hipSuccess) return 1;
    wgs->pending[wgs->n & 1] = false;
  }
  auto wgrad = [&](const void* dy, long lddy, int N1, const void* x, long ldx, int N2, int Kred, const void* gw, float alpha,
                   const void* gb) {
    pr[npr++] = emoasr_tn_problem_t{N1, N2, Kred, dy, lddy, x, ldx, (float*)gw, (long)N2, alpha, (float*)gb, alpha};
  };
  auto ln_bwd = [&](int slot, const void* dh, const void* x, const float* gamma, const float* mean, const float* rstd,
                    const void* dres, void* dx, const void* ggam, const void* gbet, void* pre, float scale, uint64_t seed) {
    emoasr_ln_bwd_opts_t o{};
    if (pre && p > 0.f) { o.dy2 = pre; o.scale2 = scale; o.drop_p2 = p; o.seed2 = seed; }
    o.defer_finalize = 1;
    return emoasr_layernorm_bwd_ex(dtype, M, d, dh, x, gamma, mean, rstd, dres, dx, (float*)ggam, (float*)gbet,
                                   io->ln_part + (long)slot * io->ln_part_stride, &o, stream);
  };
  auto dgrad = [&](int n_out, const void* dy_, const void* W, const void* Wt, void* dx_) {
    emoasr_epilogue_t e_ = plain_ep();
    if (Wt) return emoasr_gemm_nt(dtype, M, d, n_out, dy_, n_out, Wt, n_out, dx_, d, &e_, stream);
    return emoasr_gemm_nn(dtype, M, d, n_out, dy_, n_out, W, d, dx_, d, &e_, stream);
  };
  auto ffn_bwd = [&](const emoasr_ffn_params_t& P, const emoasr_ffn_params_t& Gp, const emoasr_ffn_stash_t& S, const void* x_in,
                     const void* dx_in, const void* pre_in, void* du, uint64_t s_in, const void* w1t, const void* w2t) {
    const void* dy = p > 0.f ? pre_in : dx_in;
    const float alpha = p > 0.f ? 1.f : 0.5f;
    wgrad(dy, d, d, S.a, F, F, M, Gp.w2, alpha, Gp.b2);
    emoasr_epilogue_t e = plain_ep();
    e.alpha = alpha; e.dact_pre = S.u; e.seed = s_in;
    if (g_ffn_save_dact) { e.dact = EMOASR_DACT_MUL; e.drop_p = 0.f; }
    else { e.dact = EMOASR_ACT_SWISH; e.drop_p = p; }
    if (w2t ? emoasr_gemm_nt(dtype, M, F, d, dy, d, w2t, d, du, F, &e, stream)
            : emoasr_gemm_nn(dtype, M, F, d, dy, d, P.w2, F, du, F, &e, stream)) return 1;
    wgrad(du, F, F, S.h, d, d, M, Gp.w1, 1.f, Gp.b1);
    return dgrad(F, du, P.w1, w1t, ws + bb.dh);
  };

  if (g_stack_launch && dtype == EMO_BF16) {
    emoasr_attn_t am{};
    attn_args_for(am, sv, 0, sv.n, H, d, esz, st->qkv, st->pp, st->klens, st->seed[2]);
    am.bias_u = L->bias_u; am.bias_v = L->bias_v; am.drop_p = st->p_att;
    if (g_att_bits && st->att_mask && st->p_att > 0.f) { am.keep_mask = st->att_mask; am.keep_nw = st->att_mask_nw; }
    if (emo_attn_bwd_prelaunch(dtype, &am, ws + bb.attn_ws, bb.attn_ws_bytes, (float*)(ws + bb.dpos), (long)sv.R() * d, stream)) return 1;
  }
  if (ln_bwd(0, io->dy, st->ff.y, L->fin_ln_g, st->fin_mean, st->fin_rstd, nullptr, ws + bb.dx1, G->fin_ln_g, G->fin_ln_b,
             ws + bb.pre1, 0.5f, st->seed[6])) return 1;
  if (ffn_bwd(L->ff, G->ff, st->ff, st->cv_y, ws + bb.dx1, ws + bb.pre1, ws + bb.du_ff, st->seed[5], L->ff_w1t, L->ff_w2t)) return 1;
  if (ln_bwd(1, ws + bb.dh, st->cv_y, L->ff.ln_g, st->ff.mean, st->ff.rstd, ws + bb.dx1, ws + bb.dx2, G->ff.ln_g, G->ff.ln_b,
             ws + bb.pre2, 1.f, st->seed[4])) return 1;
  {
    const void* dy = p > 0.f ? ws + bb.pre2 : ws + bb.dx2;
    wgrad(dy, d, d, st->z, d, d, M, G->pw2, 1.f, G->pw2_b);
    emoasr_epilogue_t e = plain_ep();
    if (L->pw2_t ? emoasr_gemm_nt(dtype, M, d, d, dy, d, L->pw2_t, d, ws + bb.dz, d, &e, stream)
                 : emoasr_gemm_nn(dtype, M, d, d, dy, d, L->pw2, d, ws + bb.dz, d, &e, stream)) return 1;
    if (conv_fused_ok(dtype, d)) {
      const bool conv_one_launch = sv.n > 1 && g_stack_launch;
      if (conv_one_launch &&
          emoasr_conv_module_bwd_seg(dtype, &st->seg, d, K, ws + bb.dz, st->c, st->bmean, st->bvar, L->bn_g, L->bn_b, 1e-5f,
                                     (float*)G->bn_g, (float*)G->bn_b, st->g, L->dw_w, ws + bb.dg, (float*)G->dw_w, (float*)G->dw_b,
                                     (float*)(ws + bb.bn_scr), (float*)(ws + bb.dw_scr), stream))
        return 1;
      for (int si = 0; si < sv.n && !conv_one_launch; ++si) {
        const size_t ro = (size_t)sv.row[si];
        const float *bmean = st->bmean + (size_t)si * d, *bvar = st->bvar + (size_t)si * d;
        const char* c = (const char*)st->c + ro * d * esz;
        float* tot = nullptr;
        if (emoasr_bn_swish_bwd_sums(dtype, sv.B[si] * sv.T[si], d, ws + bb.dz + ro * d * esz, c, bmean, bvar, L->bn_g, L->bn_b, 1e-5f,
                                     (float*)G->bn_g, (float*)G->bn_b, (float*)(ws + bb.bn_scr), &tot, stream)) return 1;
        if (emoasr_conv_bwd_fused(dtype, sv.B[si], sv.T[si], d, K, ws + bb.dz + ro * d * esz, c, bmean, bvar, L->bn_g, L->bn_b, 1e-5f,
                                  tot, (const char*)st->g + ro * 2 * d * esz, L->dw_w, ws + bb.dg + ro * 2 * d * esz, (float*)G->dw_w,
                                  (float*)G->dw_b, (float*)(ws + bb.dw_scr), stream)) return 1;
      }
    } else {
      const bool bn_one_launch = sv.n > 1 && g_stack_launch;
      if (bn_one_launch) {
        const RowSegs sg = row_segs_of(sv, d);
        int tmax = 0;
        for (int si = 0; si < sv.n; ++si) tmax = std::max(tmax, sv.T[si]);
        float* tot = nullptr;
        if (emo_bn_swish_bwd_sums_seg_dt(dtype, sg, d, ws + bb.dz, st->c, st->bmean, st->bvar, L->bn_g, L->bn_b, 1e-5f, (float*)G->bn_g,
                                         (float*)G->bn_b, (float*)(ws + bb.bn_scr), &tot, s)) return 1;
        if (emo_bn_bwd_apply_seg(dtype, sg, d, ws + bb.dz, st->c, st->bmean, st->bvar, L->bn_g, L->bn_b, 1e-5f, tot, ws + bb.dc, s)) return 1;
        if (emo_dwconv_seg(dtype, sg, tmax, d, K, ws + bb.dc, L->dw_w, nullptr, ws + bb.dgl, 1, nullptr, s)) return 1;
        if (emo_dwconv_bwd_w_seg(dtype, sg, tmax, d, K, ws + bb.dc, st->gl, (float*)G->dw_w, (float*)G->dw_b, (float*)(ws + bb.dw_scr), s))
          return 1;
      }
      for (int si = 0; si < sv.n && !bn_one_launch; ++si) {
        const size_t ro = (size_t)sv.row[si];
        const int B = sv.B[si], T = sv.T[si];
        const float *bmean = st->bmean + (size_t)si * d, *bvar = st->bvar + (size_t)si * d;
        if (emoasr_bn_swish_bwd(dtype, B * T, d, ws + bb.dz + ro * d * esz, (const char*)st->c + ro * d * esz, bmean, bvar, L->bn_g,
                                L->bn_b, 1e-5f, ws + bb.dc + ro * d * esz, (float*)G->bn_g, (float*)G->bn_b,
                                (float*)(ws + bb.bn_scr), stream)) return 1;
        if (emoasr_dwconv_bwd_x(dtype, B, T, d, K, ws + bb.dc + ro * d * esz, L->dw_w, ws + bb.dgl + ro * d * esz, stream)) return 1;
        if (emoasr_dwconv_bwd_w(dtype, B, T, d, K, ws + bb.dc + ro * d * esz, (const char*)st->gl + ro * d * esz, (float*)G->dw_w,
                                (float*)G->dw_b, 1, (float*)(ws + bb.dw_scr), stream)) return 1;
      }
      if (emoasr_glu_bwd(dtype, M, d, st->g, ws + bb.dgl, ws + bb.dg, stream)) return 1;
    }
    wgrad(ws + bb.dg, 2 * d, 2 * d, st->cv_h, d, d, M, G->pw1, 1.f, G->pw1_b);
    if (dgrad(2 * d, ws + bb.dg, L->pw1, L->pw1_t, ws + bb.dh)) return 1;
    if (ln_bwd(2, ws + bb.dh, st->at_y, L->cv_ln_g, st->cv_mean, st->cv_rstd, ws + bb.dx2, ws + bb.dx3, G->cv_ln_g, G->cv_ln_b,
               ws + bb.pre3, 1.f, st->seed[3])) return 1;
  }
  {
    const void* dy = p > 0.f ? ws + bb.pre3 : ws + bb.dx3;
    wgrad(dy, d, d, st->o, d, d, M, G->wout, 1.f, G->bout);
    emoasr_epilogue_t e = plain_ep();
    if (L->wout_t ? emoasr_gemm_nt(dtype, M, d, d, dy, d, L->wout_t, d, ws + bb.dout, d, &e, stream)
                  : emoasr_gemm_nn(dtype, M, d, d, dy, d, L->wout, d, ws + bb.dout, d, &e, stream)) return 1;
    if (dtype != EMO_BF16) {
      if (hipMemsetAsync(ws + bb.dpos, 0, (size_t)R * d * 4, s) != hipSuccess) return 1;
      for (int si = 0; si < sv.n; ++si) {
        const size_t ro = (size_t)sv.row[si], po = (size_t)sv.prow[si];
        char* dqkv = ws + bb.dqkv + ro * 3 * d * esz;
        emoasr_attn_t a{};
        attn_args_for(a, sv, si, si + 1, H, d, esz, st->qkv, st->pp, st->klens, st->seed[2]);
        a.bias_u = L->bias_u; a.bias_v = L->bias_v; a.drop_p = st->p_att;
        a.out = (char*)st->o + ro * d * esz; a.lse = st->lse + ro * H;
        a.dout = ws + bb.dout + ro * d * esz; a.delta = (float*)(ws + bb.delta) + ro * H;
        a.dq = dqkv; a.dk = dqkv + (size_t)d * esz; a.dv = dqkv + (size_t)2 * d * esz;
        a.dpos = (float*)(ws + bb.dpos) + po * d; a.dbias_u = (float*)G->bias_u; a.dbias_v = (float*)G->bias_v;
        if (emoasr_attn_bwd_mat_bind(dtype, &a, (char*)io->attn_img + bb.img[si], ws + bb.attn_ws)) return 1;
        if (emoasr_attn_bwd(dtype, &a, stream)) return 1;
      }
    }
    const int astep = g_stack_launch ? sv.n : 1;
    for (int si = 0; si < sv.n && dtype == EMO_BF16; si += astep) {
      const size_t ro = (size_t)sv.row[si], po = (size_t)sv.prow[si];
      const long Rs = sv.prow[si + astep] - sv.prow[si];
      char* dqkv = ws + bb.dqkv + ro * 3 * d * esz;
      emoasr_attn_t a{};
      attn_args_for(a, sv, si, si + astep, H, d, esz, st->qkv, st->pp, st->klens, st->seed[2]);
      a.bias_u = L->bias_u; a.bias_v = L->bias_v; a.drop_p = st->p_att;
      a.out = (char*)st->o + ro * d * esz; a.lse = st->lse + ro * H;
      if (g_att_bits && st->att_mask && st->p_att > 0.f) { a.keep_mask = st->att_mask + ro * H * st->att_mask_nw; a.keep_nw = st->att_mask_nw; }
      a.dout = ws + bb.dout + ro * d * esz; a.delta = (float*)(ws + bb.delta) + ro * H;
      a.dq = dqkv; a.dk = dqkv + (size_t)d * esz; a.dv = dqkv + (size_t)2 * d * esz;
      float* dpos = (float*)(ws + bb.dpos) + po * d;
      a.dpos = dpos; a.dbias_u = (float*)G->bias_u; a.dbias_v = (float*)G->bias_v;
      emo_attn_bwd_fused_extras(dpos, Rs * d, dpos, ws + bb.dpos_t + po * d * esz, Rs * d);
      emo_attn_bwd_defer_join(astep == sv.n);
      if (emoasr_attn_bwd_fused(dtype, &a, ws + bb.attn_ws, bb.attn_ws_bytes, stream)) return 1;
    }
    wgrad(dtype == EMO_BF16 ? ws + bb.dpos_t : ws + bb.dpos, d, d, st->pos_t, d, d, R, G->wpos, 1.f, nullptr);
    wgrad(ws + bb.dqkv, 3 * d, 3 * d, st->at_h, d, d, M, G->wqkv, 1.f, G->bqkv);
    if (dgrad(3 * d, ws + bb.dqkv, L->wqkv, L->wqkv_t, ws + bb.dh)) return 1;
    if (ln_bwd(3, ws + bb.dh, st->ffm.y, L->att_ln_g, st->at_mean, st->at_rstd, ws + bb.dx3, ws + bb.dx4, G->att_ln_g,
               G->att_ln_b, ws + bb.pre4, 0.5f, st->seed[1])) return 1;
  }
  if (ffn_bwd(L->ffm, G->ffm, st->ffm, st->x, ws + bb.dx4, ws + bb.pre4, ws + bb.du_ffm, st->seed[0], L->ffm_w1t, L->ffm_w2t)) return 1;
  if (ln_bwd(4, ws + bb.dh, st->x, L->ffm.ln_g, st->ffm.mean, st->ffm.rstd, ws + bb.dx4, io->dx, G->ffm.ln_g, G->ffm.ln_b,
             nullptr, 0.f, 0)) return 1;
  emo_attn_bwd_join(stream);
  if (!wgs) return emoasr_gemm_tn_grouped(dtype, npr, pr, stream);
  const int slot = wgs->n & 1;
  if (hipEventRecord(wgs->fork, s) != hipSuccess || hipStreamWaitEvent(wgs->side, wgs->fork, 0) != hipSuccess) {
    emo_set_error("conformer_layer_bwd: fork to the weight-gradient stream failed");
    return 1;
  }
  if (emoasr_gemm_tn_grouped(dtype, npr, pr, wgs->side)) return 1;
  if (hipEventRecord(wgs->done[slot], wgs->side) != hipSuccess) { emo_set_error("conformer_layer_bwd: hipEventRecord failed"); return 1; }
  wgs->pending[slot] = true;
  ++wgs->n;
  return 0;
}
```

Before: 5.945 million frames/s.

## Process strips of time tiles per block in fused conv kernels with LDS ring buffer

```diff
diff --git a/emoasr_amd/csrc/api.hip b/emoasr_amd/csrc/api.hip
--- a/emoasr_amd/csrc/api.hip
+++ b/emoasr_amd/csrc/api.hip
@@ -59,6 +59,7 @@
 void emo_gemm_set_big_korder(int v);
 void emo_gemm_set_big_min_tiles(int v);
 void emo_conv_set_dwconv_lds(int v);
+void emo_conv_set_strip(int v);
 void emo_layer_set_conv_fused(int v);
 void emo_layer_set_wgrad_side(int v);
 void emo_layer_set_stack_launch(int v);
@@ -170,6 +171,7 @@
   if (strcmp(name, "big_korder") == 0) { emo_gemm_set_big_korder(value); return 0; }
   if (strcmp(name, "big_min_tiles") == 0) { emo_gemm_set_big_min_tiles(value); return 0; }
   if (strcmp(name, "dwconv_lds") == 0) { emo_conv_set_dwconv_lds(value); return 0; }
+  if (strcmp(name, "conv_strip") == 0) { emo_conv_set_strip(value); return 0; }
   if (strcmp(name, "conv_fused") == 0) { emo_layer_set_conv_fused(value); return 0; }
   if (strcmp(name, "wgrad_side") == 0) { emo_layer_set_wgrad_side(value); return 0; }
   if (strcmp(name, "stack_launch") == 0) { emo_layer_set_stack_launch(value); return 0; }
diff --git a/emoasr_amd/csrc/convfused.hip b/emoasr_amd/csrc/convfused.hip
--- a/emoasr_amd/csrc/convfused.hip
+++ b/emoasr_amd/csrc/convfused.hip
@@ -6,7 +6,6 @@
 
 constexpr int CF_TT = 32;
 constexpr int CF_MAXK = 31;
-constexpr int CF_ROWS = CF_TT + CF_MAXK - 1;
 constexpr int CF_CB = 256;
 constexpr int CF_ROWS_P = 64;
 
@@ -20,17 +19,19 @@
   return *reinterpret_cast<const unsigned*>(base + row * CF_CB + 2 * pair);
 }
 
+__device__ __forceinline__ int ring_row(int u) { return (u & (CF_ROWS_P - 1)) * CF_CB; }
+
 template <bool GLU>
 __global__ __launch_bounds__(CF_CB) void cf_dwconv_kernel(int Tn, int C, int K, const bf16* __restrict__ x,
                                                         const float* __restrict__ w, const float* __restrict__ bias,
-                                                        bf16* __restrict__ y, int flip, float* __restrict__ part,
+                                                        bf16* __restrict__ y, int flip, float* __restrict__ part, int S,
                                                         const RowSegs sg) {
   __shared__ __attribute__((aligned(16))) bf16 zs[CF_ROWS_P * CF_CB];
   __shared__ __attribute__((aligned(16))) bf16 os[CF_TT * CF_CB];
   const int tid = threadIdx.x;
   const int cb = blockIdx.y * CF_CB;
   const int ldx = GLU ? 2 * C : C;
-  int b = blockIdx.z, nx = gridDim.x;
+  int b = blockIdx.z;
   if (sg.n > 1) {
     const int si = rowsegs_of_utt(sg, b);
     Tn = sg.T[si];
@@ -38,10 +39,12 @@
     y += sg.row[si] * C;
     if (part) part += sg.part[si];
     b -= sg.b0[si];
-    nx = (Tn + CF_TT - 1) / CF_TT;
-    if ((int)blockIdx.x >= nx) return;
-  }
-  const int t0 = blockIdx.x * CF_TT, pad = (K - 1) / 2;
+  }
+  const int nx = (Tn + CF_TT - 1) / CF_TT;
+  const int tile0 = blockIdx.x * S;
+  if (tile0 >= nx) return;
+  const int ntile = min(S, nx - tile0);
+  const int pad = (K - 1) / 2;
   const int nch = min(CF_CB, C - cb);
   const int pr = tid & (CF_CB / 2 - 1), half = tid / (CF_CB / 2);
   f2 wr[CF_MAXK];
@@ -58,36 +61,43 @@
   }
   const __amdgpu_buffer_rsrc_t rs = make_rsrc(x + (long)b * Tn * ldx);
   const int ch8 = (tid & (CF_CB / 8 - 1)) * 8;
-  {
-    Vec16<bf16> sa[CF_ROWS_P / 8], sg[GLU ? CF_ROWS_P / 8 : 1];
-#pragma unroll
-    for (int it = 0; it < CF_ROWS_P / 8; ++it) {
-      const int row = tid / (CF_CB / 8) + it * 8;
-      const int t = t0 + row - pad;
-      const bool ok = row < CF_TT + K - 1 && t >= 0 && t < Tn && ch8 < nch;
+  const int c0 = cb + 2 * pr;
+  const f2 bv = (bias && 2 * pr < nch) ? f2{bias[c0], bias[c0 + 1]} : f2{0.f, 0.f};
+  auto stage32 = [&](int t0, int u0) {
+    Vec16<bf16> sa[CF_TT / 8], sb[GLU ? CF_TT / 8 : 1];
+#pragma unroll
+    for (int it = 0; it < CF_TT / 8; ++it) {
+      const int u = u0 + tid / (CF_CB / 8) + it * 8;
+      const int t = u - pad;
+      const bool ok = u - t0 < CF_TT + K - 1 && t >= 0 && t < Tn && ch8 < nch;
       const unsigned off = ok ? (unsigned)(((long)t * ldx + cb + ch8) * 2) : EMO_OOB;
       sa[it] = buf_load16<bf16>(rs, off);
-      if constexpr (GLU) sg[it] = buf_load16<bf16>(rs, ok ? off + (unsigned)(C * 2) : EMO_OOB);
-    }
-#pragma unroll
-    for (int it = 0; it < CF_ROWS_P / 8; ++it) {
-      const int row = tid / (CF_CB / 8) + it * 8;
+      if constexpr (GLU) sb[it] = buf_load16<bf16>(rs, ok ? off + (unsigned)(C * 2) : EMO_OOB);
+    }
+#pragma unroll
+    for (int it = 0; it < CF_TT / 8; ++it) {
+      const int u = u0 + tid / (CF_CB / 8) + it * 8;
       Vec16<bf16> a = sa[it];
       if constexpr (GLU) {
 #pragma unroll
-        for (int e = 0; e < 8; ++e) a.v[e] = (bf16)((float)a.v[e] * sigmoidf_((float)sg[it].v[e]));
-      }
-      store16(&zs[row * CF_CB + ch8], a);
-    }
-  }
-  __syncthreads();
-  {
-    const int c0 = cb + 2 * pr;
+        for (int e = 0; e < 8; ++e) a.v[e] = (bf16)((float)a.v[e] * sigmoidf_((float)sb[it].v[e]));
+      }
+      store16(&zs[ring_row(u) + ch8], a);
+    }
+  };
+  for (int k = 0; k < ntile; ++k) {
+    const int tile = tile0 + k, t0 = tile * CF_TT;
+    if (k == 0) {
+      stage32(t0, t0);
+      stage32(t0, t0 + CF_TT);
+    } else {
+      stage32(t0, t0 + 2 * pad);
+    }
+    __syncthreads();
     if (2 * pr < nch) {
-      const f2 bv = bias ? f2{bias[c0], bias[c0 + 1]} : f2{0.f, 0.f};
       f2 win[CF_TT / 2 + CF_MAXK - 1];
 #pragma unroll
-      for (int i = 0; i < CF_TT / 2 + CF_MAXK - 1; ++i) win[i] = unpack2(lds_pair(zs, half * (CF_TT / 2) + i, pr));
+      for (int i = 0; i < CF_TT / 2 + CF_MAXK - 1; ++i) win[i] = unpack2(*reinterpret_cast<const unsigned*>(zs + ring_row(t0 + half * (CF_TT / 2) + i) + 2 * pr));
 #pragma unroll
       for (int i = 0; i < CF_TT / 2; ++i) {
         f2 acc = bv;
@@ -96,67 +106,78 @@
         *reinterpret_cast<unsigned*>(os + (half * (CF_TT / 2) + i) * CF_CB + 2 * pr) = pack2(acc);
       }
     }
-  }
-  __syncthreads();
-#pragma unroll
-  for (int it = 0; it < CF_TT / 8; ++it) {
-    const int row = tid / (CF_CB / 8) + it * 8;
-    if (t0 + row < Tn && ch8 < nch)
-      *reinterpret_cast<bf16x8*>(y + ((long)b * Tn + t0 + row) * C + cb + ch8) = *reinterpret_cast<const bf16x8*>(os + row * CF_CB + ch8);
-  }
-  if (part && tid < nch) {
-    float out[CF_TT];
-    float s = 0.f;
-#pragma unroll
-    for (int i = 0; i < CF_TT; ++i) {
-      out[i] = t0 + i < Tn ? (float)os[i * CF_CB + tid] : 0.f;
-      s += out[i];
-    }
-    const int n = min(CF_TT, Tn - t0);
-    const float mb = s / n;
-    float m2 = 0.f;
-#pragma unroll
-    for (int i = 0; i < CF_TT; ++i) {
-      const float d = out[i] - mb;
-      m2 += i < n ? d * d : 0.f;
-    }
-    float* p = part + ((long)b * nx + blockIdx.x) * 2 * C + cb + tid;
-    p[0] = s;
-    p[C] = m2;
-  }
-}
-
-__global__ __launch_bounds__(CF_CB) void cf_conv_bwd_kernel(int Tn, int C, int K, const bf16* __restrict__ ds,
-                                                          const bf16* __restrict__ cv, const float* __restrict__ mean,
-                                                          const float* __restrict__ var, const float* __restrict__ gamma,
-                                                          const float* __restrict__ beta, float eps,
-                                                          const float* __restrict__ tot, const bf16* __restrict__ g,
-                                                          const float* __restrict__ w, bf16* __restrict__ dg,
-                                                          float* __restrict__ wpart, const RowSegs sg) {
+    __syncthreads();
+#pragma unroll
+    for (int it = 0; it < CF_TT / 8; ++it) {
+      const int row = tid / (CF_CB / 8) + it * 8;
+      if (t0 + row < Tn && ch8 < nch)
+        *reinterpret_cast<bf16x8*>(y + ((long)b * Tn + t0 + row) * C + cb + ch8) = *reinterpret_cast<const bf16x8*>(os + row * CF_CB + ch8);
+    }
+    if (part && tid < nch) {
+      float out[CF_TT];
+      float s = 0.f;
+#pragma unroll
+      for (int i = 0; i < CF_TT; ++i) {
+        out[i] = t0 + i < Tn ? (float)os[i * CF_CB + tid] : 0.f;
+        s += out[i];
+      }
+      const int n = min(CF_TT, Tn - t0);
+      const float mb = s / n;
+      float m2 = 0.f;
+#pragma unroll
+      for (int i = 0; i < CF_TT; ++i) {
+        const float d = out[i] - mb;
+        m2 += i < n ? d * d : 0.f;
+      }
+      float* p = part + ((long)b * nx + tile) * 2 * C + cb + tid;
+      p[0] = s;
+      p[C] = m2;
+    }
+  }
+}
+
+constexpr int CF_BWD_LDS = 2 * CF_ROWS_P * CF_CB * 2 + 6 * CF_CB * 4;
+__global__ __launch_bounds__(CF_CB, 2) void cf_conv_bwd_kernel(int Tn, int C, int K, const bf16* __restrict__ ds,
+                                                             const bf16* __restrict__ cv, const float* __restrict__ mean,
+                                                             const float* __restrict__ var, const float* __restrict__ gamma,
+                                                             const float* __restrict__ beta, float eps,
+                                                             const float* __restrict__ tot, const bf16* __restrict__ g,
+                                                             const float* __restrict__ w, bf16* __restrict__ dg,
+                                                             float* __restrict__ wpart, int S, int per_tile, const RowSegs sg) {
   extern __shared__ __attribute__((aligned(16))) char smem[];
   bf16* dcs = reinterpret_cast<bf16*>(smem);
   bf16* zs = dcs + CF_ROWS_P * CF_CB;
+  float* cst = reinterpret_cast<float*>(zs + CF_ROWS_P * CF_CB);
   const int tid = threadIdx.x;
   const int cb = blockIdx.y * CF_CB;
   const int nch = min(CF_CB, C - cb);
   int b = blockIdx.z;
+  long row0 = 0;
   if (sg.n > 1) {
     const int si = rowsegs_of_utt(sg, b);
+    for (int k = 0; k < 8; ++k)
+      if (k < si) row0 += (long)(sg.b0[k + 1] - sg.b0[k]) * (((sg.T[k] + CF_TT - 1) / CF_TT + S - 1) / S);
     Tn = sg.T[si];
     ds += sg.row[si] * C; cv += sg.row[si] * C; g += sg.row[si] * 2 * C; dg += sg.row[si] * 2 * C;
     mean += (long)si * C; var += (long)si * C; tot += (long)si * 2 * C;
     b -= sg.b0[si];
-    if ((int)blockIdx.x * CF_TT >= Tn) {
-      float* p = wpart + ((long)blockIdx.z * gridDim.x + blockIdx.x) * (K + 1) * C + cb + tid;
-      if (tid < nch)
-        for (int j = 0; j <= K; ++j) p[(long)j * C] = 0.f;
-      return;
-    }
-  }
-  const int t0 = blockIdx.x * CF_TT, pad = (K - 1) / 2;
+  }
+  const int nx = (Tn + CF_TT - 1) / CF_TT;
+  const int tile0 = blockIdx.x * S;
+  if (tile0 >= nx) return;
+  const int ntile = min(S, nx - tile0);
+  row0 += per_tile ? (long)b * nx : (long)b * ((nx + S - 1) / S) + blockIdx.x;
+  const int pad = (K - 1) / 2;
   const int ch8 = (tid & (CF_CB / 8 - 1)) * 8;
   const bool chok = ch8 < nch;
-  const int pr = tid & (CF_CB / 2 - 1), half = tid / (CF_CB / 2);
+  const int pr = tid & (CF_CB / 2 - 1), half = __builtin_amdgcn_readfirstlane(tid / (CF_CB / 2));
+  {
+    const int cc = cb + tid;
+    const bool ok = tid < nch;
+    cst[0 * CF_CB + tid] = ok ? mean[cc] : 0.f; cst[1 * CF_CB + tid] = ok ? rsqrtf(var[cc] + eps) : 0.f;
+    cst[2 * CF_CB + tid] = ok ? gamma[cc] : 0.f; cst[3 * CF_CB + tid] = ok ? beta[cc] : 0.f;
+    cst[4 * CF_CB + tid] = ok ? tot[cc] : 0.f; cst[5 * CF_CB + tid] = ok ? tot[C + cc] : 0.f;
+  }
   f2 wr[CF_MAXK];
   {
     float* wsm = reinterpret_cast<float*>(smem);
@@ -167,54 +188,47 @@
       wr[j] = (j < K && 2 * pr < nch) ? f2{wsm[(2 * pr) * K + (K - 1 - j)], wsm[(2 * pr + 1) * K + (K - 1 - j)]} : f2{0.f, 0.f};
     __syncthreads();
   }
-  {
-    const __amdgpu_buffer_rsrc_t rsd = make_rsrc(ds + (long)b * Tn * C), rsc = make_rsrc(cv + (long)b * Tn * C);
-    const __amdgpu_buffer_rsrc_t rsg = make_rsrc(g + (long)b * Tn * 2 * C);
-    {
-      Vec16<bf16> ga[CF_ROWS_P / 8], gb[CF_ROWS_P / 8];
-#pragma unroll
-      for (int it = 0; it < CF_ROWS_P / 8; ++it) {
-        const int row = tid / (CF_CB / 8) + it * 8;
-        const int t = t0 + row - pad;
-        const bool ok = row < CF_TT + K - 1 && t >= 0 && t < Tn && chok;
-        const unsigned goff = ok ? (unsigned)(((long)t * 2 * C + cb + ch8) * 2) : EMO_OOB;
-        ga[it] = buf_load16<bf16>(rsg, goff);
-        gb[it] = buf_load16<bf16>(rsg, ok ? goff + (unsigned)(C * 2) : EMO_OOB);
-      }
-#pragma unroll
-      for (int it = 0; it < CF_ROWS_P / 8; ++it) {
-        const int row = tid / (CF_CB / 8) + it * 8;
-        const int core = row - pad;
-        (void)core;
-        Vec16<bf16> z;
-#pragma unroll
-        for (int e = 0; e < 8; ++e) z.v[e] = (bf16)((float)ga[it].v[e] * sigmoidf_((float)gb[it].v[e]));
-        store16(&zs[row * CF_CB + ch8], z);
-      }
-    }
-    float mu[8], is[8], gm[8], bt[8], m1[8], m2[8];
-#pragma unroll
-    for (int j = 0; j < 8; ++j) {
-      const int cc = cb + ch8 + j;
-      mu[j] = chok ? mean[cc] : 0.f; is[j] = chok ? rsqrtf(var[cc] + eps) : 0.f;
-      gm[j] = chok ? gamma[cc] : 0.f; bt[j] = chok ? beta[cc] : 0.f;
-      m1[j] = chok ? tot[cc] : 0.f; m2[j] = chok ? tot[C + cc] : 0.f;
-    }
-    Vec16<bf16> dvs[CF_ROWS_P / 8], yvs[CF_ROWS_P / 8];
-#pragma unroll
-    for (int it = 0; it < CF_ROWS_P / 8; ++it) {
-      const int row = tid / (CF_CB / 8) + it * 8;
-      const int t = t0 + row - pad;
-      const bool ok = row < CF_TT + K - 1 && t >= 0 && t < Tn && chok;
+  const __amdgpu_buffer_rsrc_t rsd = make_rsrc(ds + (long)b * Tn * C), rsc = make_rsrc(cv + (long)b * Tn * C);
+  const __amdgpu_buffer_rsrc_t rsg = make_rsrc(g + (long)b * Tn * 2 * C);
+  auto stage32 = [&](int t0, int u0) {
+    Vec16<bf16> ga[CF_TT / 8], gb[CF_TT / 8], dvs[CF_TT / 8], yvs[CF_TT / 8];
+#pragma unroll
+    for (int it = 0; it < CF_TT / 8; ++it) {
+      const int u = u0 + tid / (CF_CB / 8) + it * 8;
+      const int t = u - pad;
+      const bool ok = u - t0 < CF_TT + K - 1 && t >= 0 && t < Tn && chok;
+      const unsigned goff = ok ? (unsigned)(((long)t * 2 * C + cb + ch8) * 2) : EMO_OOB;
+      ga[it] = buf_load16<bf16>(rsg, goff);
+      gb[it] = buf_load16<bf16>(rsg, ok ? goff + (unsigned)(C * 2) : EMO_OOB);
+    }
+#pragma unroll
+    for (int it = 0; it < CF_TT / 8; ++it) {
+      const int u = u0 + tid / (CF_CB / 8) + it * 8;
+      Vec16<bf16> z;
+#pragma unroll
+      for (int e = 0; e < 8; ++e) z.v[e] = (bf16)((float)ga[it].v[e] * sigmoidf_((float)gb[it].v[e]));
+      store16(&zs[ring_row(u) + ch8], z);
+    }
+#pragma unroll
+    for (int it = 0; it < CF_TT / 8; ++it) {
+      const int u = u0 + tid / (CF_CB / 8) + it * 8;
+      const int t = u - pad;
+      const bool ok = u - t0 < CF_TT + K - 1 && t >= 0 && t < Tn && chok;
       const unsigned off = ok ? (unsigned)(((long)t * C + cb + ch8) * 2) : EMO_OOB;
       dvs[it] = buf_load16<bf16>(rsd, off);
       yvs[it] = buf_load16<bf16>(rsc, off);
     }
-#pragma unroll
-    for (int it = 0; it < CF_ROWS_P / 8; ++it) {
-      const int row = tid / (CF_CB / 8) + it * 8;
-      const int t = t0 + row - pad;
-      const bool ok = row < CF_TT + K - 1 && t >= 0 && t < Tn && chok;
+    float mu[8], is[8], gm[8], bt[8], m1[8], m2[8];
+#pragma unroll
+    for (int j = 0; j < 8; ++j) {
+      mu[j] = cst[0 * CF_CB + ch8 + j]; is[j] = cst[1 * CF_CB + ch8 + j]; gm[j] = cst[2 * CF_CB + ch8 + j];
+      bt[j] = cst[3 * CF_CB + ch8 + j]; m1[j] = cst[4 * CF_CB + ch8 + j]; m2[j] = cst[5 * CF_CB + ch8 + j];
+    }
+#pragma unroll
+    for (int it = 0; it < CF_TT / 8; ++it) {
+      const int u = u0 + tid / (CF_CB / 8) + it * 8;
+      const int t = u - pad;
+      const bool ok = u - t0 < CF_TT + K - 1 && t >= 0 && t < Tn && chok;
       const Vec16<bf16> dv = dvs[it], yv = yvs[it];
       Vec16<bf16> o;
 #pragma unroll
@@ -223,67 +237,127 @@
         const float dbn = (float)dv.v[e] * dswishf_(gm[e] * xh + bt[e]);
         o.v[e] = ok ? (bf16)(gm[e] * is[e] * (dbn - m1[e] - xh * m2[e])) : (bf16)0.f;
       }
-      store16(&dcs[row * CF_CB + ch8], o);
-    }
-  }
-  __syncthreads();
-  if (2 * pr >= nch) return;
+      store16(&dcs[ring_row(u) + ch8], o);
+    }
+  };
+  const bool active = 2 * pr < nch;
   const int c0 = cb + 2 * pr;
-  {
-    f2 dcw[CF_TT / 2 + CF_MAXK - 1];
-#pragma unroll
-    for (int i = 0; i < CF_TT / 2 + CF_MAXK - 1; ++i) dcw[i] = unpack2(lds_pair(dcs, half * (CF_TT / 2) + i, pr));
-    bf16* dgb = dg + (long)b * Tn * 2 * C + c0;
-#pragma unroll
-    for (int i = 0; i < CF_TT / 2; ++i) {
-      f2 acc = f2{0.f, 0.f};
-#pragma unroll
-      for (int j = 0; j < CF_MAXK; ++j) acc = emo_mac2(wr[j], dcw[i + j], acc);
-      const f2 d = unpack2(pack2(acc));
-      const int fr = half * (CF_TT / 2) + i;
-      const bool fok = t0 + fr < Tn;
-      const bf16* gp = g + ((long)b * Tn + (fok ? t0 + fr : 0)) * 2 * C + c0;
-      const f2 a = fok ? unpack2(*reinterpret_cast<const unsigned*>(gp)) : f2{0.f, 0.f};
-      const f2 gt = fok ? unpack2(*reinterpret_cast<const unsigned*>(gp + C)) : f2{0.f, 0.f};
-      const f2 sg = f2{sigmoidf_(gt[0]), sigmoidf_(gt[1])};
-      if (t0 + fr < Tn) {
-        *reinterpret_cast<unsigned*>(dgb + (long)(t0 + fr) * 2 * C) = pack2(d * sg);
-        *reinterpret_cast<unsigned*>(dgb + (long)(t0 + fr) * 2 * C + C) = pack2(d * a * sg * (f2{1.f, 1.f} - sg));
-      }
-    }
-  }
-  {
-    constexpr int TAPS = (CF_MAXK + 1) / 2;
-    const int j0 = half * TAPS;
-    f2 dcc[CF_TT];
-#pragma unroll
-    for (int i = 0; i < CF_TT; ++i) dcc[i] = unpack2(lds_pair(dcs, i + pad, pr));
-    f2 zw[CF_TT + TAPS - 1];
-#pragma unroll
-    for (int i = 0; i < CF_TT + TAPS - 1; ++i) zw[i] = j0 + i < CF_ROWS_P ? unpack2(lds_pair(zs, j0 + i, pr)) : f2{0.f, 0.f};
-    f2 acc[TAPS];
-#pragma unroll
-    for (int j = 0; j < TAPS; ++j) acc[j] = f2{0.f, 0.f};
-    f2 sb = f2{0.f, 0.f};
-#pragma unroll
-    for (int i = 0; i < CF_TT; ++i) {
-      const f2 d = dcc[i];
-      sb += d;
-#pragma unroll
-      for (int j = 0; j < TAPS; ++j) acc[j] = emo_mac2(d, zw[i + j], acc[j]);
-    }
-    const long blk = ((long)blockIdx.z * gridDim.x + blockIdx.x);
-    float* p = wpart + blk * (K + 1) * C + c0;
-#pragma unroll
-    for (int j = 0; j < TAPS; ++j)
-      if (j0 + j < K) *reinterpret_cast<f2*>(p + (long)(j0 + j) * C) = acc[j];
-    if (half == 0) *reinterpret_cast<f2*>(p + (long)K * C) = sb;
+  constexpr int TAPS = (CF_MAXK + 1) / 2;
+  const int j0 = half * TAPS;
+  f2 acc[TAPS];
+#pragma unroll
+  for (int j = 0; j < TAPS; ++j) acc[j] = f2{0.f, 0.f};
+  f2 sb = f2{0.f, 0.f};
+  for (int k = 0; k < ntile; ++k) {
+    const int t0 = (tile0 + k) * CF_TT;
+    if (k == 0) {
+      stage32(t0, t0);
+      stage32(t0, t0 + CF_TT);
+    } else {
+      __syncthreads();
+      stage32(t0, t0 + 2 * pad);
+    }
+    __syncthreads();
+    if (active) {
+    {
+      auto dcrow = [&](int i) { return unpack2(*reinterpret_cast<const unsigned*>(dcs + ring_row(t0 + half * (CF_TT / 2) + i) + 2 * pr)); };
+      f2 dcw[CF_TT / 2 + CF_MAXK - 1];
+#pragma unroll
+      for (int i = 0; i < CF_MAXK - 1; ++i) dcw[i] = dcrow(i);
+      bf16* dgb = dg + (long)b * Tn * 2 * C + c0;
+#pragma unroll
+      for (int i = 0; i < CF_TT / 2; ++i) {
+        if (i % 8 == 0) {
+          if (i) __builtin_amdgcn_sched_barrier(0);
+#pragma unroll
+          for (int e = 0; e < 8; ++e) dcw[CF_MAXK - 1 + i + e] = dcrow(CF_MAXK - 1 + i + e);
+        }
+        f2 a2 = f2{0.f, 0.f};
+#pragma unroll
+        for (int j = 0; j < CF_MAXK; ++j) a2 = emo_mac2(wr[j], dcw[i + j], a2);
+        const f2 d = unpack2(pack2(a2));
+        const int fr = half * (CF_TT / 2) + i;
+        const bool fok = t0 + fr < Tn;
+        const bf16* gp = g + ((long)b * Tn + (fok ? t0 + fr : 0)) * 2 * C + c0;
+        const f2 a = fok ? unpack2(*reinterpret_cast<const unsigned*>(gp)) : f2{0.f, 0.f};
+        const f2 gt = fok ? unpack2(*reinterpret_cast<const unsigned*>(gp + C)) : f2{0.f, 0.f};
+        const f2 sgm = f2{sigmoidf_(gt[0]), sigmoidf_(gt[1])};
+        if (fok) {
+          *reinterpret_cast<unsigned*>(dgb + (long)(t0 + fr) * 2 * C) = pack2(d * sgm);
+          *reinterpret_cast<unsigned*>(dgb + (long)(t0 + fr) * 2 * C + C) = pack2(d * a * sgm * (f2{1.f, 1.f} - sgm));
+        }
+      }
+    }
+    {
+      auto zrow = [&](int i) { return unpack2(*reinterpret_cast<const unsigned*>(zs + ring_row(t0 + j0 + i) + 2 * pr)); };
+      f2 zw[CF_TT + TAPS - 1];
+#pragma unroll
+      for (int i = 0; i < TAPS - 1; ++i) zw[i] = zrow(i);
+#pragma unroll
+      for (int c = 0; c < CF_TT / 8; ++c) {
+        f2 dcc[8];
+#pragma unroll
+        for (int i = 0; i < 8; ++i) {
+          zw[8 * c + TAPS - 1 + i] = zrow(8 * c + TAPS - 1 + i);
+          dcc[i] = unpack2(*reinterpret_cast<const unsigned*>(dcs + ring_row(t0 + 8 * c + i + pad) + 2 * pr));
+        }
+#pragma unroll
+        for (int i = 0; i < 8; ++i) {
+          const f2 d = dcc[i];
+          sb += d;
+#pragma unroll
+          for (int j = 0; j < TAPS; ++j) acc[j] = emo_mac2(d, zw[8 * c + i + j], acc[j]);
+        }
+        __builtin_amdgcn_sched_barrier(0);
+      }
+    }
+    if (per_tile || k == ntile - 1) {
+      float* p = wpart + (row0 + (per_tile ? tile0 + k : 0)) * (K + 1) * C + c0;
+#pragma unroll
+      for (int j = 0; j < TAPS; ++j) {
+        if (j0 + j < K) *reinterpret_cast<f2*>(p + (long)(j0 + j) * C) = acc[j];
+        acc[j] = f2{0.f, 0.f};
+      }
+      if (half == 0) *reinterpret_cast<f2*>(p + (long)K * C) = sb;
+      sb = f2{0.f, 0.f};
+    }
+    }
   }
 }
 
 }
 
 int emo_dwconv_bwd_w_reduce(int nblk, int C, int K, const float* part, float* dw, float* dbias, hipStream_t s);
+
+static int g_conv_strip = 0;
+void emo_conv_set_strip(int v) { g_conv_strip = v > 0 ? std::min(v, 1 << 16) : 0; }
+namespace {
+long live_strips(int n, const int* B, const int* T, int S) {
+  long r = 0;
+  for (int i = 0; i < n; ++i) r += (long)B[i] * cdiv(cdiv(T[i], CF_TT), S);
+  return r;
+}
+int strip_tiles(int n, const int* B, const int* T, int cy) {
+  if (g_conv_strip > 0) return g_conv_strip;
+  static int cus = 0;
+  if (!cus) {
+    int dev = 0, v = 0;
+    cus = (hipGetDevice(&dev) == hipSuccess && hipDeviceGetAttribute(&v, hipDeviceAttributeMultiprocessorCount, dev) == hipSuccess && v > 0) ? v : 256;
+  }
+  int S = 1;
+  while (S < 8 && live_strips(n, B, T, S) * cy > 2L * cus) ++S;
+  return S;
+}
+int bwd_lds_attr() {
+  static bool done = false;
+  if (!done) {
+    hipError_t e = hipFuncSetAttribute((const void*)cf_conv_bwd_kernel, hipFuncAttributeMaxDynamicSharedMemorySize, CF_BWD_LDS);
+    if (e != hipSuccess) { emo_set_error("hipFuncSetAttribute(%d): %s", CF_BWD_LDS, hipGetErrorString(e)); return 1; }
+    done = true;
+  }
+  return 0;
+}
+}
 
 extern "C" int emoasr_glu_dwconv_fwd(int dtype, int B, int Tn, int C, int K, const void* g, const float* w,
                                      const float* bias, void* c, float* part, void* stream) {
@@ -291,16 +365,18 @@
   EMO_CHECK(K <= CF_MAXK && (K & 1) && C % 8 == 0, "glu_dwconv_fwd: K=%d (odd, <= %d), C=%d (multiple of 8)", K, CF_MAXK, C);
   EMO_CHECK((long)Tn * 2 * C * 2 < (1L << 32), "glu_dwconv_fwd: utterance larger than 4 GiB");
   if (B * Tn == 0) return 0;
-  dim3 grid(cdiv(Tn, CF_TT), cdiv(C, CF_CB), B);
-  cf_dwconv_kernel<true><<<grid, CF_CB, 0, (hipStream_t)stream>>>(Tn, C, K, (const bf16*)g, w, bias, (bf16*)c, 0, part, RowSegs{});
+  const int S = strip_tiles(1, &B, &Tn, cdiv(C, CF_CB));
+  dim3 grid(cdiv(cdiv(Tn, CF_TT), S), cdiv(C, CF_CB), B);
+  cf_dwconv_kernel<true><<<grid, CF_CB, 0, (hipStream_t)stream>>>(Tn, C, K, (const bf16*)g, w, bias, (bf16*)c, 0, part, S, RowSegs{});
   EMO_LAUNCH_CHECK();
   return 0;
 }
 
 int emo_dwconv_lds(int B, int Tn, int C, int K, const void* x, const float* w, const float* bias, void* y, int flip,
                    float* part, hipStream_t s) {
-  dim3 grid(cdiv(Tn, CF_TT), cdiv(C, CF_CB), B);
-  cf_dwconv_kernel<false><<<grid, CF_CB, 0, s>>>(Tn, C, K, (const bf16*)x, w, bias, (bf16*)y, flip, part, RowSegs{});
+  const int S = strip_tiles(1, &B, &Tn, cdiv(C, CF_CB));
+  dim3 grid(cdiv(cdiv(Tn, CF_TT), S), cdiv(C, CF_CB), B);
+  cf_dwconv_kernel<false><<<grid, CF_CB, 0, s>>>(Tn, C, K, (const bf16*)x, w, bias, (bf16*)y, flip, part, S, RowSegs{});
   EMO_LAUNCH_CHECK();
   return 0;
 }
@@ -315,21 +391,16 @@
   EMO_CHECK(scratch != nullptr && tot != nullptr, "conv_bwd_fused: scratch and tot are required");
   if (B * Tn == 0) return 0;
   hipStream_t s = (hipStream_t)stream;
-  constexpr int bytes = 2 * CF_ROWS_P * CF_CB * 2;
-  static bool attr_done = false;
-  if (!attr_done) {
-    hipError_t e = hipFuncSetAttribute((const void*)cf_conv_bwd_kernel, hipFuncAttributeMaxDynamicSharedMemorySize, bytes);
-    if (e != hipSuccess) { emo_set_error("hipFuncSetAttribute(%d): %s", bytes, hipGetErrorString(e)); return 1; }
-    attr_done = true;
-  }
-  dim3 grid(cdiv(Tn, CF_TT), cdiv(C, CF_CB), B);
-  cf_conv_bwd_kernel<<<grid, CF_CB, bytes, s>>>(Tn, C, K, (const bf16*)ds, (const bf16*)cv, mean, var, gamma, beta, eps, tot,
-                                              (const bf16*)g, w, (bf16*)dg, scratch, RowSegs{});
+  if (bwd_lds_attr()) return 1;
+  const int S = strip_tiles(1, &B, &Tn, cdiv(C, CF_CB));
+  dim3 grid(cdiv(cdiv(Tn, CF_TT), S), cdiv(C, CF_CB), B);
+  cf_conv_bwd_kernel<<<grid, CF_CB, CF_BWD_LDS, s>>>(Tn, C, K, (const bf16*)ds, (const bf16*)cv, mean, var, gamma, beta, eps, tot,
+                                                   (const bf16*)g, w, (bf16*)dg, scratch, S, 1, RowSegs{});
   EMO_LAUNCH_CHECK();
-  return emo_dwconv_bwd_w_reduce(grid.x * B, C, K, scratch, dw, dbias, s);
-}
-
-int emo_bn_stats_finalize_seg(const RowSegs& sg, int C, const float* part, float* mean, float* var, float* running_mean,
+  return emo_dwconv_bwd_w_reduce(cdiv(Tn, CF_TT) * B, C, K, scratch, dw, dbias, s);
+}
+
+int emo_bn_stats_finalize_seg(const RowSegs& sg, int C, float* part, float* mean, float* var, float* running_mean,
                               float* running_var, float momentum, long long* nbt, hipStream_t s);
 int emo_bn_swish_fwd_seg(const RowSegs& sg, int C, const void* y, const float* mean, const float* var, const float* gamma,
                          const float* beta, float eps, void* z, hipStream_t s);
@@ -370,8 +441,9 @@
   EMO_CHECK(!training || (part && bmean && bvar), "conv_module_fwd_seg: training needs the BatchNorm buffers");
   hipStream_t s = (hipStream_t)stream;
   EmoTimerScope timer_(EMO_TIMER_CONV_MODULE, s, 0.0, 5.0 * (double)sg.row[sg.n] * C * 2.0);
-  dim3 grid(cdiv(tmax, CF_TT), cdiv(C, CF_CB), sg.b0[sg.n]);
-  cf_dwconv_kernel<true><<<grid, CF_CB, 0, s>>>(tmax, C, K, (const bf16*)g, w, bias, (bf16*)c, 0, training ? part : nullptr, sg);
+  const int S = strip_tiles(seg->n, seg->B, seg->T, cdiv(C, CF_CB));
+  dim3 grid(cdiv(cdiv(tmax, CF_TT), S), cdiv(C, CF_CB), sg.b0[sg.n]);
+  cf_dwconv_kernel<true><<<grid, CF_CB, 0, s>>>(tmax, C, K, (const bf16*)g, w, bias, (bf16*)c, 0, training ? part : nullptr, S, sg);
   EMO_LAUNCH_CHECK();
   if (training) {
     if (emo_bn_stats_finalize_seg(sg, C, part, bmean, bvar, running_mean, running_var, momentum, num_batches_tracked, s)) return 1;
@@ -404,16 +476,11 @@
   EmoTimerScope timer_(EMO_TIMER_CONV_MODULE, s, 0.0, 8.0 * (double)sg.row[sg.n] * C * 2.0);
   float* tot = nullptr;
   if (emo_bn_swish_bwd_sums_seg(sg, C, dz, c, bmean, bvar, gamma, beta, eps, dgamma, dbeta, bn_scratch, &tot, s)) return 1;
-  constexpr int bytes = 2 * CF_ROWS_P * CF_CB * 2;
-  static bool attr_done = false;
-  if (!attr_done) {
-    hipError_t e = hipFuncSetAttribute((const void*)cf_conv_bwd_kernel, hipFuncAttributeMaxDynamicSharedMemorySize, bytes);
-    if (e != hipSuccess) { emo_set_error("hipFuncSetAttribute(%d): %s", bytes, hipGetErrorString(e)); return 1; }
-    attr_done = true;
-  }
-  dim3 grid(cdiv(tmax, CF_TT), cdiv(C, CF_CB), sg.b0[sg.n]);
-  cf_conv_bwd_kernel<<<grid, CF_CB, bytes, s>>>(tmax, C, K, (const bf16*)dz, (const bf16*)c, bmean, bvar, gamma, beta, eps, tot,
-                                              (const bf16*)g, w, (bf16*)dg, dw_scratch, sg);
+  if (bwd_lds_attr()) return 1;
+  const int S = strip_tiles(seg->n, seg->B, seg->T, cdiv(C, CF_CB));
+  dim3 grid(cdiv(cdiv(tmax, CF_TT), S), cdiv(C, CF_CB), sg.b0[sg.n]);
+  cf_conv_bwd_kernel<<<grid, CF_CB, CF_BWD_LDS, s>>>(tmax, C, K, (const bf16*)dz, (const bf16*)c, bmean, bvar, gamma, beta, eps, tot,
+                                                   (const bf16*)g, w, (bf16*)dg, dw_scratch, S, 0, sg);
   EMO_LAUNCH_CHECK();
-  return emo_dwconv_bwd_w_reduce(grid.x * sg.b0[sg.n], C, K, dw_scratch, dw, dbias, s);
-}
+  return emo_dwconv_bwd_w_reduce((int)live_strips(seg->n, seg->B, seg->T, S), C, K, dw_scratch, dw, dbias, s);
+}
diff --git a/emoasr_amd/csrc/convmodule.hip b/emoasr_amd/csrc/convmodule.hip
--- a/emoasr_amd/csrc/convmodule.hip
+++ b/emoasr_amd/csrc/convmodule.hip
@@ -71,7 +71,7 @@
   EmoScratch* tsc_ = emo_stream_scratch(EMO_SCRATCH_BN_TICKETS, (void*)(stream_), 2 * 64 * sizeof(unsigned)); \
   if (!tsc_) return 1;                                                                            \
   unsigned* tickets_ = static_cast<unsigned*>(tsc_->dev)
-__global__ __launch_bounds__(1024) void bn_stats_finalize_kernel(int B_, int Tn_, int C, const float* __restrict__ part_,
+__global__ __launch_bounds__(1024) void bn_stats_finalize_kernel(int B_, int Tn_, int C, float* __restrict__ part_,
                                                                  float* __restrict__ mean_, float* __restrict__ var_,
                                                                  float* __restrict__ running_mean,
                                                                  float* __restrict__ running_var, float momentum,
@@ -84,7 +84,7 @@
   const int c = blockIdx.x * BNF_CH + lane;
   const int ns = sg.n > 1 ? sg.n : 1, si = blockIdx.y;
   const int B = sg.n > 1 ? sg.b0[si + 1] - sg.b0[si] : B_, Tn = sg.n > 1 ? sg.T[si] : Tn_;
-  const float* part = sg.n > 1 ? part_ + sg.part[si] : part_;
+  float* part = sg.n > 1 ? part_ + sg.part[si] : part_;
   float* mean = mean_ + (long)si * C;
   float* var = var_ + (long)si * C;
   const int nx = (Tn + DW_TT - 1) / DW_TT, nblk = B * nx;
@@ -121,6 +121,7 @@
     for (int g = 0; g < BNF_G; ++g) m2sum += red[g][lane];
     mean[c] = mu;
     var[c] = m2sum / M;
+    if (sg.n > 1) part[c] = m2sum;
   }
   if (!running_mean && !running_var && !num_batches_tracked) return;
   __syncthreads();
@@ -136,8 +137,7 @@
     for (int k = 0; k < ns; ++k) {
       const float Mk = sg.n > 1 ? (float)(sg.row[k + 1] - sg.row[k]) : M;
       const float mk = __hip_atomic_load(mean_ + (long)k * C + c, __ATOMIC_RELAXED, __HIP_MEMORY_SCOPE_AGENT);
-      const float vk = __hip_atomic_load(var_ + (long)k * C + c, __ATOMIC_RELAXED, __HIP_MEMORY_SCOPE_AGENT);
-      const float m2k = k == si ? m2sum : vk * Mk;
+      const float m2k = k == si ? m2sum : __hip_atomic_load(part_ + sg.part[k] + c, __ATOMIC_RELAXED, __HIP_MEMORY_SCOPE_AGENT);
       rm = (1.f - momentum) * rm + momentum * (k == si ? mu : mk);
       rv = (1.f - momentum) * rv + momentum * (Mk > 1.f ? m2k / (Mk - 1.f) : m2k / Mk);
     }
@@ -511,7 +511,7 @@
   EMO_CHECK(B * Tn > 0, "bn_stats_finalize: empty batch");
   EMO_CHECK(cdiv(C, BNF_CH) <= 64, "bn_stats_finalize: C=%d too wide for the ticket table", C);
   EMO_BN_TICKETS(stream);
-  bn_stats_finalize_kernel<<<cdiv(C, BNF_CH), 1024, 0, (hipStream_t)stream>>>(B, Tn, C, part, mean, var, running_mean,
+  bn_stats_finalize_kernel<<<cdiv(C, BNF_CH), 1024, 0, (hipStream_t)stream>>>(B, Tn, C, const_cast<float*>(part), mean, var, running_mean,
                                                                           running_var, momentum, num_batches_tracked, RowSegs{}, tickets_);
   EMO_LAUNCH_CHECK();
   return 0;
@@ -622,7 +622,7 @@
   return 0;
 }
 
-int emo_bn_stats_finalize_seg(const RowSegs& sg, int C, const float* part, float* mean, float* var, float* running_mean,
+int emo_bn_stats_finalize_seg(const RowSegs& sg, int C, float* part, float* mean, float* var, float* running_mean,
                               float* running_var, float momentum, long long* nbt, hipStream_t s) {
   EMO_CHECK(cdiv(C, BNF_CH) <= 64, "bn_stats_finalize: C=%d too wide for the ticket table", C);
   EMO_BN_TICKETS(s);
diff --git a/emoasr_amd/csrc/layer.hip b/emoasr_amd/csrc/layer.hip
--- a/emoasr_amd/csrc/layer.hip
+++ b/emoasr_amd/csrc/layer.hip
@@ -11,7 +11,7 @@
 void emo_attn_bwd_join(void* stream);
 int emo_attn_bwd_prelaunch(int dtype, const emoasr_attn_t* a, void* ws, size_t ws_bytes, float* zero, long zn, void* stream);
 
-int emo_bn_stats_finalize_seg(const RowSegs& sg, int C, const float* part, float* mean, float* var, float* running_mean,
+int emo_bn_stats_finalize_seg(const RowSegs& sg, int C, float* part, float* mean, float* var, float* running_mean,
                               float* running_var, float momentum, long long* nbt, hipStream_t s);
 int emo_bn_swish_fwd_seg_dt(int dtype, const RowSegs& sg, int C, const void* y, const float* mean, const float* var,
                             const float* gamma, const float* beta, float eps, void* z, hipStream_t s);
```

After: 6.055 million frames/s (median of 6 runs). +1.8%, better.
